# volume-em/empanada-napari

Measured on AMD Instinct MI355X. Metric: EM tiles/sec (1024^2 fp16), higher is better.
Workload: dtype f16

## Files before the change

### empanada-napari_amd/_abi.py

```python
import ctypes as C
import os

from . import build as _build

_lib = None

c_int, c_i32, c_i64, c_f32, c_f64 = C.c_int, C.c_int32, C.c_int64, C.c_float, C.c_double
vp, cp, sz = C.c_void_p, C.c_char_p, C.c_size_t


class PdlConfig(C.Structure):
    _fields_ = [
        ('num_classes', c_i32), ('stage4_stride', c_i32), ('decoder_channels', c_i32),
        ('aspp_channels', c_i32), ('n_stages', c_i32), ('low_level_stages', c_i32 * 3),
        ('low_level_proj_sem', c_i32 * 3), ('low_level_proj_ins', c_i32 * 3),
        ('atrous_rates', c_i32 * 3), ('ins_decoder', c_i32), ('num_fc', c_i32),
        ('subdivision_num_points', c_i32), ('arch', c_i32), ('fpn_dim', c_i32), ('fpn_layers', c_i32),
        ('encoder', c_i32), ('rn_stem', c_i32), ('rn_widths', c_i32 * 4), ('rn_depths', c_i32 * 4),
        ('rn_groups', c_i32 * 4), ('rn_strides', c_i32 * 4), ('rn_se', c_i32),
    ]


PROTOTYPES = {
    'emp_last_error': (cp, []),
# ... 13 lines not shown
    'emp_pdl_forward_padded': (c_int, [vp, vp, c_int, c_f32, c_f32, c_int, c_int, c_int, c_int, c_int, c_int, c_int, vp,
                                       vp, vp, vp]),
    'emp_pdl_flops': (c_f64, [vp, c_int, c_int, c_int, c_int]),
    'emp_pdl_profile': (c_int, [vp, c_int]),
    'emp_pdl_profile_read': (c_int, [vp, C.POINTER(c_f64), C.POINTER(c_f64), C.POINTER(c_int)]),
    'emp_pdl_tap': (c_int, [vp, cp, C.POINTER(vp), C.POINTER(c_i64)]),
    'emp_pdl_num_taps': (c_int, [vp]),
    'emp_pdl_tap_raw': (c_int, [vp, cp, C.POINTER(vp), C.POINTER(c_i64)]),
    'emp_pdl_tap_name': (cp, [vp, c_int]),
    'emp_copy_d2d': (c_int, [vp, vp, sz, vp]),
    'emp_conv2d_nhwc_f16': (c_int, [vp, c_int, c_int, c_int, c_int, c_int, vp, vp, vp, vp, c_int, vp, c_int, c_int,
                                    c_int, c_int, c_int, c_int, c_int, c_int, c_int, vp]),
    'emp_conv256_pack_weights': (c_int, [vp, vp, c_int, c_int, c_int, c_int, vp]),
    'emp_conv2d_grouped_nhwc_f32': (c_int, [vp, c_int, c_int, c_int, c_int, c_int, c_int, c_int, vp, vp, vp, c_int, c_int, c_int,
                                            c_int, c_int, c_int, c_int, c_int, vp]),
    'emp_conv2d_nhwc_f32': (c_int, [vp, c_int, c_int, c_int, c_int, c_int, vp, vp, vp, vp, c_int, vp, c_int, c_int,
                                    c_int, c_int, c_int, c_int, c_int, c_int, vp]),
    'emp_conv2d_nhwc_f16x3': (c_int, [vp, c_int, c_int, c_int, c_int, c_int, vp, vp, vp, vp, c_int, vp, c_int, c_int,
                                      c_int, c_int, c_int, c_int, c_int, c_int, c_int, c_int, vp]),
    'emp_conv2d_nhwc_f16x3_ex': (c_int, [vp, c_int, c_int, c_int, c_int, c_int, vp, vp, vp, vp, c_int, vp, c_int, c_int, c_int,
                                         c_int, c_int, c_int, c_int, c_int, c_int, c_int, vp, c_int, c_int, c_int, c_int, c_int,
                                         vp, vp, c_int, vp, vp]),
    'emp_sepconv_x3_pack': (c_int, [vp, vp, c_int, c_int, c_int, vp, vp, vp]),
    'emp_sepconv_x3_nhwc_f32': (c_int, [vp, c_int, c_int, c_int, c_int, c_int, vp, vp, vp, c_int, c_int, vp, c_int, vp, vp, c_int, vp,
                                        c_int, vp]),
    'emp_hl32_from_f32': (c_int, [vp, vp, c_i64, c_int, c_int, c_int, vp]),
    'emp_hl32_to_f32': (c_int, [vp, vp, c_i64, c_int, c_int, c_int, vp]),
    'emp_x3p_pack_weights': (c_int, [vp, vp, c_int, c_int, vp]),
    'emp_conv2d_hl32_f16x3': (c_int, [vp, c_int, c_int, c_int, c_int, c_int, vp, vp, vp, vp, c_int, c_int, vp, c_int, c_int, c_int,
                                      c_int, c_int, c_int, c_int, c_int, c_int, vp]),
    'emp_conv2d_hl32_f16x3_ksplit': (c_int, [vp, c_int, c_int, c_int, c_int, c_int, vp, vp, vp, vp, c_int, c_int, vp, c_int, c_int, vp, c_int, c_int,
                                             c_int, c_int, c_int, c_int, c_int, c_int, c_int, vp, c_i64, vp]),
    'emp_conv1x1_dual_nhwc_f16': (c_int, [vp, c_int, c_int, c_int, c_int, c_int, vp, c_int, c_int, c_int, c_int, c_int, vp, vp, vp,
                                  c_int, c_int, c_int, c_int, vp]),
    'emp_dwconv_nhwc_f16': (c_int, [vp, c_int, c_int, c_int, c_int, c_int, vp, c_int, vp, c_int, vp]),
    'emp_sepconv5x5_pack_pw': (c_int, [vp, c_int, c_int, c_int, vp, vp]),
    'emp_sepconv5x5_nhwc_f16': (c_int, [vp, c_int, c_int, c_int, c_int, c_int, vp, vp, vp, c_int, c_int, vp,
                                        c_int, vp, vp, c_int, vp, vp]),
    'emp_sepconvp_pack_dw': (c_int, [vp, c_int, c_int, vp, vp]),
    'emp_sepconvp_pack_pw': (c_int, [vp, c_int, c_int, c_int, vp, vp]),
    'emp_sepconvp_nhwc_f16': (c_int, [vp, c_int, c_int, c_int, c_int, c_int, c_int, vp, vp, vp, c_int, c_int, vp,
                                      c_int, vp, vp, c_int, vp, vp]),
    'emp_sepconvp_ws_pack_pw': (c_int, [vp, c_int, c_int, c_int, vp, vp]),
    'emp_sepconvp_ws_nhwc_f16': (c_int, [vp, c_int, c_int, c_int, c_int, c_int, c_int, vp, vp, vp, c_int, c_int, vp,
                                         c_int, vp, vp, c_int, vp, vp]),
    'emp_sepconv3x3_nhwc_f16': (c_int, [vp, c_int, c_int, c_int, c_int, c_int, vp, vp, vp, c_int, c_int, vp, c_int, vp]),
    'emp_sm_create': (vp, [c_i64, c_i64, c_f64, c_f64, c_int]),
    'emp_sm_destroy': (None, [vp]),
    'emp_sm_push_slice_runs': (c_int, [vp, vp, c_i64, c_i64, c_i64]),
    'emp_sm_push_slices_runs': (c_int, [vp, c_i64, vp, vp, c_i64, c_i64]),
    'emp_sm_push_slice_objects': (c_int, [vp, c_i64, vp, vp, vp, vp, vp]),
    'emp_sm_num_slices': (c_i64, [vp]),
    'emp_lsa_maximize': (c_int, [vp, c_i64, c_i64, vp, vp]),
    'emp_lsa_maximize_sparse': (c_int, [c_i64, c_i64, c_i64, vp, vp, vp, vp, vp]),
    'emp_sm_prepare': (c_int, [vp, c_i64, c_i64]),
    'emp_sm_state_size': (c_int, [vp, c_i64, vp, vp]),
    'emp_sm_export_state': (c_int, [vp, c_i64, vp, vp, vp, vp]),
    'emp_sm_import_state': (c_int, [vp, c_i64, c_i64, vp, vp, vp, c_i64, c_int]),
    'emp_sm_begin_backward': (c_int, [vp]),
    'emp_sm_step_begin': (c_int, [vp, c_i64, C.POINTER(c_int), C.POINTER(c_int)]),
    'emp_sm_iou': (vp, [vp]),
    'emp_sm_step_apply': (c_int, [vp, vp, vp, c_i64]),
    'emp_sm_run': (c_int, [vp, c_i64, c_int, c_i64, c_int, vp]),
    'emp_sm_solver_stats': (c_int, [vp, C.POINTER(c_i64), C.POINTER(c_i64)]),
    'emp_sm_pending_shape': (c_int, [vp, vp, vp]),
    'emp_sm_tracker_init': (c_int, [vp, c_int, c_i64, c_i64, c_i64]),
    'emp_sm_track': (c_int, [vp, c_i64, c_i64]),
    'emp_sm_track_range': (c_int, [vp, c_i64, c_i64, c_i64]),
    'emp_sm_tracker_finish': (c_int, [vp]),
    'emp_sm_num_tracks': (c_i64, [vp]),
    'emp_sm_track_info': (c_int, [vp, c_i64, C.POINTER(c_i64), C.POINTER(c_i64), C.POINTER(c_i64)]),
    'emp_sm_track_runs': (c_int, [vp, c_i64, vp, vp]),
    'emp_sm_tracks_info': (c_int, [vp, vp, vp, vp, C.POINTER(c_i64)]),
    'emp_sm_tracks_runs': (c_int, [vp, vp, vp]),
    'emp_sm_slice_num_objects': (c_i64, [vp, c_i64]),
    'emp_sm_slice_object_info': (c_int, [vp, c_i64, c_i64, C.POINTER(c_i64), C.POINTER(c_i64), C.POINTER(c_i64)]),
    'emp_sm_slice_object_runs': (c_int, [vp, c_i64, c_i64, vp, vp]),
    'emp_logits_to_prob': (c_int, [vp, vp, c_int, c_int, c_int, c_int, vp]),
    'emp_median_slices': (c_int, [C.POINTER(vp), c_int, vp, sz, vp]),
    'emp_median_recursive': (c_int, [vp, vp, c_int, c_int, c_int, vp, sz, vp]),
    'emp_instance_cells_work_bytes': (sz, [c_int, c_int, c_int]),
    'emp_instance_cells': (c_int, [vp, vp, c_int, c_int, c_int, c_f32, c_int, c_int, c_int, vp, vp, vp, c_int, vp, vp]),
    'emp_panoptic_merge_work_bytes': (sz, [c_int, c_int, c_int]),
    'emp_ccl8_work_bytes': (sz, [c_int, c_int, c_int]),
    'emp_ccl8': (c_int, [vp, c_int, c_int, c_int, vp, vp, vp, vp]),
    'emp_force_connected_work_bytes': (sz, [c_int, c_int, c_int]),
    'emp_force_connected': (c_int, [vp, c_int, c_int, c_int, C.POINTER(c_i32), c_int, c_i64, vp, vp, vp]),
    'emp_ccl26': (c_int, [vp, c_int, c_int, c_int, vp, vp, vp, vp]),
    'emp_morph_cross3d': (c_int, [vp, vp, c_int, c_int, c_int, c_int, vp]),
    'emp_fill_holes_slices': (c_int, [vp, c_i64, c_i64, c_i64]),
    'emp_rle_extract_work_bytes': (sz, [c_int, c_int, c_int]),
    'emp_rle_extract': (c_int, [vp, c_int, c_int, c_int, vp, vp, c_int, vp, vp]),
    'emp_ccl_range': (c_int, [vp, c_int, c_int, c_int, c_int, c_int, c_i64, c_i64, vp, vp, vp, vp]),
    'emp_rle_extract_range': (c_int, [vp, c_int, c_int, c_int, c_int, c_i64, c_i64, vp, vp, c_int, vp, vp]),
    'emp_rle_fill': (c_int, [vp, vp, vp, c_i64, vp, c_i64, c_int, vp]),
    'emp_rle_fill_ordered': (c_int, [vp, vp, vp, vp, c_i64, vp, c_i64, c_int, vp, vp]),
    'emp_rle_pair_intersections': (c_int, [vp, vp, vp, vp, c_i64, vp]),
    'emp_ranges_vote': (c_int, [vp, c_i64, c_int, vp, C.POINTER(c_i64)]),
    'emp_gather_segments_i64': (c_int, [vp, vp, vp, vp, vp, vp, c_i64, vp, vp]),
    'emp_panoptic_merge': (c_int, [vp, vp, c_int, c_int, c_int, c_int, c_f32, C.POINTER(c_i32), c_int, c_i64, c_i64,
                                   c_i64, c_int, vp, vp, vp]),
    'emp_label_overlap_work_bytes': (sz, [c_i64]),
    'emp_label_overlap_reset': (c_int, [vp, c_i64, vp]),
    'emp_label_overlap_accumulate': (c_int, [vp, c_int, vp, c_int, c_i64, vp, c_i64, vp, C.POINTER(c_int)]),
    'emp_label_overlap_grow': (c_int, [vp, c_i64, vp, c_i64, vp, C.POINTER(c_int)]),
    'emp_label_overlap_finalize': (c_int, [vp, c_i64, vp, vp, c_i64, C.POINTER(c_i64), vp]),
    'emp_overlap_match': (c_int, [c_i64, vp, vp, vp, c_int, vp, vp, C.POINTER(c_i64), vp, vp, C.POINTER(c_i64), vp, vp, vp, vp,
                                  C.POINTER(c_i64)]),
    'emp_label_table_work_bytes': (sz, [c_i64]),
    'emp_label_table_reset': (c_int, [vp, c_i64, vp]),
    'emp_label_table_accumulate': (c_int, [vp, c_int, c_i64, c_int, c_int, c_int, c_int, vp, c_i64, vp, C.POINTER(c_int)]),
    'emp_label_table_grow': (c_int, [vp, c_i64, vp, c_i64, vp, C.POINTER(c_int)]),
    'emp_label_table_finalize': (c_int, [vp, c_i64, vp, vp, vp, c_i64, C.POINTER(c_i64), vp]),
    'emp_label_map_build': (c_int, [vp, vp, c_i64, vp, vp, c_i64, vp]),
    'emp_label_apply_map': (c_int, [vp, c_int, vp, c_int, vp, c_i64, c_int, c_int, c_int, c_int, vp, vp, c_i64, vp]),
    'emp_morph_tile_shape': (c_int, [c_int, c_int, c_int, C.POINTER(c_int), C.POINTER(c_int), C.POINTER(c_int)]),
    'emp_morph_labels': (c_int, [vp, c_int, c_int, c_int, c_int, c_int, c_int, c_int, vp, vp, c_i64, vp, vp, c_int, vp, c_i64, vp,
                                 C.POINTER(c_int)]),
    'emp_fill_holes_tile_shape': (c_int, [c_int, C.POINTER(c_int), C.POINTER(c_int), C.POINTER(c_int)]),
    'emp_fill_holes_labels': (c_int, [vp, c_int, c_int, c_int, c_int, c_int, c_int, c_i64, vp, vp, vp, c_i64, vp, vp, c_int, vp, vp, c_i64,
                                      vp, C.POINTER(c_int)]),
}


class EmpError(RuntimeError):
    pass


def lib_path():
    return _build.LIB


def load(build_if_missing=False):
    global _lib
    if _lib is not None:
        return _lib
    import torch
    path = lib_path()
    if not os.path.exists(path):
        if build_if_missing:
            _build.build_all()
        else:
            raise EmpError(f'{path} not found: run `python __graft_entry__.py` (build()) first; '
                           'the HIP engine has no CPU fallback')
    lib = C.CDLL(path)
    for name, (res, args) in PROTOTYPES.items():
        try:
            fn = getattr(lib, name)
        except AttributeError as e:
            raise EmpError(f'{path} does not export {name}') from e
        fn.restype = res
        fn.argtypes = args
    _lib = lib
    return lib


def check(rc, what=''):
    if rc != 0:
        msg = load().emp_last_error()
        raise EmpError(f'{what} failed ({rc}): {msg.decode() if msg else "?"}')


def ptr(t):
    return None if t is None else C.c_void_p(t.data_ptr())


# ... 4 lines not shown
```

### empanada-napari_amd/csrc/abi.hip

```cpp
#include <stdarg.h>

#include <map>
#include <mutex>
#include <utility>
#include <vector>

#include "common.h"

namespace emp {

static thread_local char g_err[1024] = "no error";

void set_error(const char* fmt, ...) {
  va_list ap;
  va_start(ap, fmt);
  vsnprintf(g_err, sizeof(g_err), fmt, ap);
  va_end(ap);
}

const void* zero_page() {
  static void* page = nullptr;
  static std::once_flag once;
  std::call_once(once, [] {
    if (hipMalloc(&page, 2048) != hipSuccess) { page = nullptr; return; }
    if (hipMemset(page, 0, 2048) != hipSuccess) { (void)hipFree(page); page = nullptr; }
  });
  return page;
}

int ensure_dyn_lds(const void* kernel, int bytes) {
  static std::mutex mu;
  static std::map<std::pair<int, const void*>, int> done;
  int dev = 0;
  EMP_CHECK_HIP(hipGetDevice(&dev));
  std::lock_guard<std::mutex> lk(mu);
  auto it = done.find({dev, kernel});
  if (it != done.end() && it->second >= bytes) return EMP_OK;
  EMP_CHECK_HIP(hipFuncSetAttribute(kernel, hipFuncAttributeMaxDynamicSharedMemorySize, bytes));
  done[{dev, kernel}] = bytes;
  return EMP_OK;
}

}

using namespace emp;

extern "C" {

const char* emp_last_error(void) { return g_err; }
int emp_abi_version(void) { return 5; }

int emp_device_count(void) {
  int n = 0;
  hipError_t e = hipGetDeviceCount(&n);
  if (e != hipSuccess) {
    set_error("hipGetDeviceCount: %s", hipGetErrorString(e));
    return EMP_ERR_HIP;
  }
  return n;
}

int emp_copy_d2d(void* d_dst, const void* d_src, size_t bytes, void* stream) {
  EMP_REQUIRE(d_dst && d_src, "copy_d2d: null pointer");
  EMP_CHECK_HIP(hipMemcpyAsync(d_dst, d_src, bytes, hipMemcpyDeviceToDevice, (hipStream_t)stream));
  return EMP_OK;
}

int emp_conv2d_nhwc_f16(const void* d_in, int N, int H, int W, int Cin, int in_ld, const void* d_w,
                        const float* d_bias, const float* d_bias_n, const void* d_res, int res_ld, void* d_out,
                        int out_ld, int Cout, int KH, int KW, int stride, int pad, int dil, int relu, int variant,
                        void* stream) {
  EMP_REQUIRE(d_in && d_w && d_out, "conv2d: null pointer");
  EMP_REQUIRE(N > 0 && H > 0 && W > 0 && KH > 0 && KW > 0 && stride > 0 && dil > 0 && pad >= 0, "conv2d: bad geometry");
  EMP_REQUIRE(variant >= 0 && (variant & 15) <= 3 && ((variant >> 4) & 15) <= 7 && ((variant >> 8) & 255) <= 64 && (variant >> 16) <= 31, "conv2d: bad variant %d", variant);
  ConvParams p{};
  p.in = (const half_t*)d_in;
  p.wgt = (const half_t*)d_w;
  p.bias = d_bias;
  p.bias_n = d_bias_n;
  p.res = (const half_t*)d_res;
  p.res_ld = res_ld;
  p.out = (half_t*)d_out;
  p.zero = (const half_t*)zero_page();
  EMP_REQUIRE(p.zero != nullptr, "conv2d: could not allocate the zero page");
  p.N = N; p.H = H; p.W = W; p.Cin = Cin; p.in_ld = in_ld;
  p.Cout = Cout; p.KH = KH; p.KW = KW; p.stride = stride; p.pad = pad; p.dil = dil;
  p.Ho = (H + 2 * pad - dil * (KH - 1) - 1) / stride + 1;
  p.Wo = (W + 2 * pad - dil * (KW - 1) - 1) / stride + 1;
  EMP_REQUIRE(p.Ho > 0 && p.Wo > 0, "conv2d: empty output");
  p.out_ld = out_ld;
  p.act = relu;
  p.ps_cout = 0;
  p.M = N * p.Ho * p.Wo;
  return launch_conv_igemm(p, variant, (hipStream_t)stream);
}

int emp_conv256_pack_weights(const void* d_w, void* d_packed, int Cout, int KT, int Cin, int Cin2, void* stream) {
  return conv256_pack_weights((const half_t*)d_w, (half_t*)d_packed, Cout, KT, Cin, Cin2, (hipStream_t)stream);
}

int emp_conv2d_nhwc_f32(const float* d_in, int N, int H, int W, int Cin, int in_ld, const float* d_w, const float* d_bias,
                        const float* d_bias_n, const float* d_res, int res_ld, float* d_out, int out_ld, int Cout, int KH,
                        int KW, int stride, int pad, int dil, int act, void* stream) {
  EMP_REQUIRE(d_in && d_w && d_out, "conv2d_f32: null pointer");
  EMP_REQUIRE(N > 0 && H > 0 && W > 0 && KH > 0 && KW > 0 && stride > 0 && dil > 0 && pad >= 0, "conv2d_f32: bad geometry");
  Conv32 p{};
  p.in = d_in; p.in_ld = in_ld; p.w = d_w; p.bias = d_bias; p.bias_n = d_bias_n; p.res = d_res; p.res_ld = res_ld;
  p.out = d_out; p.out_ld = out_ld;
  p.N = N; p.H = H; p.W = W; p.Cin = Cin; p.Cout = Cout; p.KH = KH; p.KW = KW; p.stride = stride; p.pad = pad; p.dil = dil;
  p.Ho = (H + 2 * pad - dil * (KH - 1) - 1) / stride + 1;
  p.Wo = (W + 2 * pad - dil * (KW - 1) - 1) / stride + 1;
  EMP_REQUIRE(p.Ho > 0 && p.Wo > 0 && out_ld >= Cout && (d_res == nullptr || res_ld >= Cout), "conv2d_f32: bad output geometry");
  p.act = act;
  return launch_conv32(p, (hipStream_t)stream);
}

int emp_conv2d_nhwc_f16x3(const float* d_in, int N, int H, int W, int Cin, int in_ld, const float* d_w, const float* d_bias,
                          const float* d_bias_n, const float* d_res, int res_ld, float* d_out, int out_ld, int Cout, int KH,
                          int KW, int stride, int pad, int dil, int act, int groups, int cin_g, void* stream) {
  EMP_REQUIRE(d_in && d_w && d_out, "conv2d_f16x3: null pointer");
  EMP_REQUIRE(N > 0 && H > 0 && W > 0 && KH > 0 && KW > 0 && stride > 0 && dil > 0 && pad >= 0 && groups >= 1, "conv2d_f16x3: bad geometry");
  Conv32 p{};
  p.in = d_in; p.in_ld = in_ld; p.w = d_w; p.bias = d_bias; p.bias_n = d_bias_n; p.res = d_res; p.res_ld = res_ld;
  p.out = d_out; p.out_ld = out_ld;
  p.N = N; p.H = H; p.W = W; p.Cin = Cin; p.Cout = Cout; p.KH = KH; p.KW = KW; p.stride = stride; p.pad = pad; p.dil = dil;
  p.Ho = (H + 2 * pad - dil * (KH - 1) - 1) / stride + 1;
  p.Wo = (W + 2 * pad - dil * (KW - 1) - 1) / stride + 1;
  EMP_REQUIRE(p.Ho > 0 && p.Wo > 0 && out_ld >= groups * Cout && (d_res == nullptr || res_ld >= Cout), "conv2d_f16x3: bad output geometry");
  p.act = act;
  p.x3 = 1;
  if (groups > 1) { p.groups = groups; p.cin_g = cin_g; }
  return launch_conv32(p, (hipStream_t)stream);
}

int emp_conv2d_nhwc_f16x3_ex(const float* d_in, int N, int H, int W, int Cin, int in_ld, const float* d_w, const float* d_bias,
                             const float* d_bias_n, const float* d_res, int res_ld, void* d_out, int out_ld, int out_fmt, int Cout, int KH,
                             int KW, int stride, int pad, int dil, int act, int wmode, const float* d_in2, int H2, int W2, int Cin2,
                             int in2_ld, int stride2, const float* d_head_w, const float* d_head_b, int head_c, float* d_head_out,
                             void* stream) {
  EMP_REQUIRE(d_in && d_w && (d_out || d_head_w), "conv2d_f16x3_ex: null pointer");
  EMP_REQUIRE(N > 0 && H > 0 && W > 0 && KH > 0 && KW > 0 && stride > 0 && dil > 0 && pad >= 0 && wmode >= 0 && (wmode & 3) <= 2 && wmode < 8,
              "conv2d_f16x3_ex: bad geometry (wmode 0 fp32 weights, 1 split pairs, 2 pairs + LDS-DMA image; + 4: split-K allowed)");
  const bool ksplit = (wmode & 4) != 0;
  wmode &= 3;
  hipStream_t s = (hipStream_t)stream;
  Conv32 p{};
  p.in = d_in; p.in_ld = in_ld; p.w = d_w; p.bias = d_bias; p.bias_n = d_bias_n; p.res = d_res; p.res_ld = res_ld;
  p.out = (float*)d_out; p.out_ld = out_ld; p.out_fmt = out_fmt;
// ... 238 lines not shown
```

### empanada-napari_amd/csrc/common.h

```cpp
#pragma once
#include <hip/hip_runtime.h>
#include <stdint.h>
#include <stdio.h>
#include <string>

#include "../../include/empanada_hip.h"

typedef _Float16 half_t;
typedef _Float16 f16x8 __attribute__((ext_vector_type(8)));
typedef _Float16 f16x4 __attribute__((ext_vector_type(4)));
typedef _Float16 f16x2 __attribute__((ext_vector_type(2)));
typedef float f32x4 __attribute__((ext_vector_type(4)));

namespace emp {

void set_error(const char* fmt, ...);

#define EMP_CHECK_HIP(expr)                                                        \
  do {                                                                             \
    hipError_t _e = (expr);                                                        \
    if (_e != hipSuccess) {                                                        \
      emp::set_error("%s:%d: %s -> %s", __FILE__, __LINE__, #expr, hipGetErrorString(_e)); \
      return EMP_ERR_HIP;                                                          \
    }                                                                              \
// ... 88 lines not shown
int launch_sepconv5(const half_t* in, int N, int H, int W, int C, int in_ld, const half_t* dww, const half_t* pww_packed,
                    const float* bias, int Cout, int act, half_t* out, int out_ld, const float* head_w,
                    const float* head_b, int head_c, float* hout, int64_t plane, const half_t* zero, hipStream_t s,
                    int ks = 5);
bool sepconvp_supported(int C, int Cout, int head_c);
bool sepconvp_wsplit_supported(int Cout);
int launch_sepconvp_pack_pw(const float* w, int pw_ld, int C, int Cout, half_t* packed, hipStream_t s, int wsplit = 0);
int launch_sepconvp_pack_dw(const float* w, int ks, int C, float* packed, hipStream_t s);
int launch_sepconvp(const half_t* in, int N, int H, int W, int C, int in_ld, const float* dww_packed, const half_t* pww_packed,
                    const float* bias, int Cout, int act, half_t* out, int out_ld, const float* head_w,
                    const float* head_b, int head_c, float* hout, int64_t plane, const half_t* zero, hipStream_t s,
                    int ks = 5, int wsplit = 0);
int launch_head1x1(const half_t* in, int N, int P, int K, int in_ld, const float* w, const float* b, int C,
                   float* out, int64_t plane_size, const int32_t* scatter_idx, hipStream_t s);
int launch_bilinear_ac_f32_nchw(const float* in, int NC, int h, int w, float* out, int scale, hipStream_t s);
int launch_zero(void* p, size_t bytes, hipStream_t s);

struct Conv32 {
  const float* in; int in_ld;
  const float* w; const float* bias; const float* bias_n;
  const float* res; int res_ld;
  float* out; int out_ld;
  int N, H, W, Cin, Cout, KH, KW, stride, pad, dil, Ho, Wo;
  int act;
  int ps_cout;
  int groups;
  int cin_g;
  int x3;
  const float* in2; int in2_ld, Cin2, H2, W2, stride2;
  const float* head_w; float* head_part; int head_c;
  int x3_mt, x3_nt, x3_mtx;
  const float* zero;
  const uint32_t* wpair;
  const half_t* wimg;
  int in_fmt, out_fmt, res_fmt;
  const half_t* wimgp;
  float* out2; int out2_ld, split2;
  int x3p_kg;
  float* kpart; int64_t kpart_bytes; int ksplit, x3_ksteps;
};
constexpr int64_t X3_KPART_BYTES = 64ll << 20;
int launch_conv32(const Conv32& p, hipStream_t s);
int launch_conv16x3(const Conv32& p, hipStream_t s);
int launch_split_pairs(const float* w, uint32_t* out, int64_t n, hipStream_t s);
int64_t x3_weight_image_halfs(int Cout, int K, int Cin);
int launch_x3_weight_image(const float* w, half_t* out, int Cout, int K, hipStream_t s);
bool conv16x3p_supported(const Conv32& p);
int launch_conv16x3p(const Conv32& p, hipStream_t s);
int64_t x3p_image_halfs(int Cout, int K);
int x3p_kgroup(int KT, int Cin);
int launch_x3p_pack(const float* w, half_t* out, int Cout, int K, hipStream_t s, int KT = 0, int Cin = 0, int kg = 0);
int launch_hl32_from_f32(const float* in, half_t* out, int64_t rows, int C, int in_ld, int out_ld, hipStream_t s);
int launch_hl32_to_f32(const half_t* in, float* out, int64_t rows, int C, int in_ld, int out_ld, hipStream_t s);
int launch_avgpool_hl32(const half_t* in, int N, int HW, int C, int in_ld, float* out, hipStream_t s);
bool sepconv_x3_supported(int C, int Cout, int head_c, int ks);
int64_t sepx3_pw_halfs(int C, int Cout);
int launch_sepx3_pack_pw(const float* w, int pw_ld, int C, int Cout, half_t* packed, hipStream_t s);
int launch_sepx3_pack_dw(const float* w , int ks, int C, int ld, float* packed, hipStream_t s);
int launch_sepconv_x3(const float* in, int N, int H, int W, int C, int in_ld, const float* dww, const half_t* pww, const float* bias,
                      int Cout, int act, float* out, int out_ld, const float* head_w, const float* head_b, int head_c, float* hout,
                      int64_t plane, hipStream_t s, int ks = 5);
int conv16x3_cout_tiles(int Cout);
int launch_head_finish_f32(const float* part, int tiles, int N, int P, int C, const float* b, float* out, hipStream_t s);
int launch_stem3x3s2_f32(const void* img, int dtype, float sub, float mul, int N, int H, int W, int vh, int vw,
                         const float* w , const float* b, int C, float* out, int out_ld, hipStream_t s);
int launch_gate_mul_f32(float* x, int x_ld, const float* g, int g_ld, int64_t rows, int C, hipStream_t s);
int launch_stem7x7_f32(const void* img, int dtype, float sub, float mul, int N, int H, int W, int vh, int vw,
                       const float* w , const float* b , float* out, hipStream_t s);
int launch_maxpool3x3s2_f32(const float* in, int N, int H, int W, int C, float* out, hipStream_t s);
int launch_dwconv_f32(const float* in, int N, int H, int W, int C, int in_ld, const float* w , int K, float* out,
                      int out_ld, hipStream_t s);
int launch_bilinear_ac_f32_nhwc(const float* in, int N, int h, int w, int C, int in_ld, float* out, int H, int W, int out_ld,
                                hipStream_t s);
int launch_avgpool_f32(const float* in, int N, int HW, int C, int in_ld, float* out, hipStream_t s);
int launch_fuse_combine_f32(const float* a, const float* b, const float* c, float ca, float cb, float cc, int mode, int N,
                            int H, int W, int C, float* out, hipStream_t s);
int launch_head1x1_f32(const float* in, int N, int P, int K, int in_ld, const float* w, const float* b, int C, float* out,
                       int64_t plane_size, const int32_t* scatter_idx, hipStream_t s);
int launch_point_features_f32(const float* feat, int N, int fh, int fw, int C, int feat_ld, const float* coarse, int ncls,
                              const int32_t* idx, int P, int H2, int W2, float* x0, float* x1, int ld, hipStream_t s);

size_t topk_work_bytes(int N, int64_t plane);
int launch_upsample2x_keys(const float* in, int N, int C, int h, int w, float* out, uint32_t* keys, hipStream_t s);
int launch_topk_smallest(const uint32_t* keys, int N, int64_t plane, int k, void* work, size_t work_bytes,
                         int32_t* idx_out, hipStream_t s);
int launch_point_features(const half_t* feat, int N, int fh, int fw, int C, int feat_ld, const float* coarse,
                          int ncls, const int32_t* idx, int P, int H2, int W2, half_t* x0, half_t* x1, int ld,
                          hipStream_t s);

bool pr_mlp_supported(int C, int ld, int ncls, int num_fc);
int launch_pr_mlp(const half_t* feat, int N, int fh, int fw, int C, int feat_ld, const float* coarse, int ncls,
                  const int32_t* idx, int P, int H2, int W2, const half_t* const* fc_w, const float* const* fc_b,
                  int num_fc, int ld, const float* pred_w, const float* pred_b, float* out, int64_t plane, hipStream_t s);


}
```

### empanada-napari_amd/csrc/pdl_net.hip

```cpp
#include <string.h>

#include <array>
#include <map>
#include <memory>
#include <string>
#include <vector>

#include "common.h"

namespace emp {

namespace {

struct HostParam {
  std::vector<int64_t> shape;
  std::vector<float> w, b;
  bool set = false;
};

struct Act {
  half_t* p = nullptr;
  int N = 0, H = 0, W = 0, C = 0, ld = 0;
  size_t off = 0;
};
// ... 5 lines not shown
  int cout = 0, cin = 0, cin_pad = 0, kh = 1, kw = 1;
  int cin2 = 0, cin2_pad = 0;
  bool wsplit = false;
};

inline int round_up(int a, int b) { return (a + b - 1) / b * b; }

}
}

using namespace emp;

struct emp_pdl {
  emp_pdl_config cfg;
  int aspp_ch = 256, dec_ch = 256, ncls = 1;
  std::vector<std::string> param_names;
  std::map<std::string, HostParam> params;
  bool finalized = false;
  FILE* layer_log = [] { const char* e = getenv("EMP_LAYER_LOG"); return e ? fopen(e, "w") : (FILE*)nullptr; }();
  bool fuse_stem = [] { const char* e = getenv("EMP_FUSE_STEM"); return !(e && e[0] == '0'); }();
  bool fuse_ds = [] { const char* e = getenv("EMP_FUSE_DS"); return !(e && e[0] == '0'); }();
  bool fuse_b2b = [] { const char* e = getenv("EMP_FUSE_B2B"); return !(e && e[0] == '0'); }();
  bool pack256 = [] { const char* e = getenv("EMP_CONV256_PACK"); return !(e && e[0] == '0'); }();
  bool fuse_proj = [] { const char* e = getenv("EMP_FUSE_PROJ"); return !(e && e[0] == '0'); }();
  bool fuse_aspp = [] { const char* e = getenv("EMP_FUSE_ASPP"); return !(e && e[0] == '0'); }();
  bool fuse_sepconv = [] { const char* e = getenv("EMP_FUSE_SEPCONV"); return !(e && e[0] == '0'); }();
  bool fuse_pr = [] { const char* e = getenv("EMP_FUSE_PR"); return !(e && e[0] == '0'); }();
  int precise_sepconv = [] { const char* e = getenv("EMP_PRECISE_SEPCONV"); return e ? atoi(e) : 1; }();
  bool precise_wsplit = [] { const char* e = getenv("EMP_PRECISE_WSPLIT"); return !(e && e[0] == '0'); }();
  bool precise_fsplit = [] { const char* e = getenv("EMP_PRECISE_FSPLIT"); return !(e && e[0] == '0'); }();
  int sepconv_min_tiles = [] { const char* e = getenv("EMP_SEPCONV_MIN_TILES"); return e ? atoi(e) : 256; }();

  int precision = [] {
    const char* e = getenv("EMP_PRECISION");
    if (e && (!strcmp(e, "fp16") || !strcmp(e, "16"))) return 0;
    if (e && (!strcmp(e, "fp32") || !strcmp(e, "32"))) return 1;
    return 2;
  }();
  bool fp32_graph() const { return precision != 0; }
  bool x3_fuse_ds = [] { const char* e = getenv("EMP_X3_FUSE_DS"); return !(e && e[0] == '0'); }();
  bool x3_fuse_head = [] { const char* e = getenv("EMP_X3_FUSE_HEAD"); return !(e && e[0] == '0'); }();
  bool x3_planes = [] { const char* e = getenv("EMP_X3_PLANES"); return !(e && e[0] == '0'); }();
  int x3_planes_min_tiles = [] { const char* e = getenv("EMP_X3_PLANES_MIN_TILES"); return e ? atoi(e) : 128; }();
  bool x3_planes_ready = false;
  bool x3_ksplit = [] { const char* e = getenv("EMP_X3_KSPLIT"); return !(e && e[0] == '0'); }();
  float* x3_kpart = nullptr;
  bool x3_small_aspp = [] { const char* e = getenv("EMP_X3_SMALL_ASPP"); return !(e && e[0] == '0'); }();
  bool x3_fuse_stem = [] { const char* e = getenv("EMP_X3_FUSE_STEM"); return !(e && e[0] == '0'); }();
  bool x3_merge_proj = [] { const char* e = getenv("EMP_X3_MERGE_PROJ"); return !(e && e[0] == '0'); }();
  bool x3_merge_aspp = [] { const char* e = getenv("EMP_X3_MERGE_ASPP"); return !(e && e[0] == '0'); }();
  bool x3_fuse_sep = [] { const char* e = getenv("EMP_X3_FUSE_SEP"); return !(e && e[0] == '0'); }();
  int x3_sep_min_tiles = [] { const char* e = getenv("EMP_X3_SEP_MIN_TILES"); return e ? atoi(e) : 1; }();
  struct SepX3 { float* dw = nullptr; half_t* pw = nullptr; int C = 0, Cout = 0, ks = 0; };
  std::map<std::string, SepX3> sepx3;
  bool regnet_grouped = [] { const char* e = getenv("EMP_REGNET_GROUPED"); return !(e && e[0] == '0'); }();
  int64_t regnet_group_tiles = [] { const char* e = getenv("EMP_REGNET_GROUP_TILES"); return e ? atoll(e) : 2048ll; }();
  struct W32 { float* w = nullptr; float* b = nullptr; int cout = 0, cin = 0, cin16 = 0, kh = 1, kw = 1; uint32_t* wp = nullptr; int cin2 = 0, cin2_16 = 0; half_t* wimg = nullptr; half_t* wimgp = nullptr; int x3p_kg = 0; };
  std::map<std::string, W32> w32;
  std::map<std::string, std::pair<float*, size_t>> pool32;
  std::map<std::string, std::array<int, 4>> geom32;

  std::map<std::string, DevConv> convs;
  std::map<std::string, float*> f32w;
  std::map<std::string, half_t*> f16w;
  std::map<std::string, std::vector<float>> fusew;
  std::vector<void*> owned;

  char* arena = nullptr;
  size_t arena_cap = 0, arena_used = 0;
  int pN = 0, pH = 0, pW = 0, pRS = 0;
  int capN = 0;
  std::map<std::string, Act> acts;
  std::vector<std::string> act_order;
  std::map<std::string, std::pair<size_t, size_t>> raw;
  double flops = 0.0;
  size_t image_bytes = 0;
  bool profile = false;
  std::vector<std::pair<hipEvent_t, hipEvent_t>> prof_events;
  size_t prof_used = 0;
  double prof_flops = 0.0;
  int64_t par_limit = [] { const char* e = getenv("EMP_PAR_DECODERS"); return e ? atoll(e) : (int64_t)4 << 20; }();
  hipStream_t aux = nullptr;
  hipEvent_t ev_fork = nullptr, ev_join = nullptr;

  ~emp_pdl() {
    for (void* p : owned) (void)hipFree(p);
    for (auto& kv : pool32) (void)hipFree(kv.second.first);
    if (arena) (void)hipFree(arena);
    if (layer_log) fclose(layer_log);
    for (auto& e : prof_events) { (void)hipEventDestroy(e.first); (void)hipEventDestroy(e.second); }
    if (ev_fork) (void)hipEventDestroy(ev_fork);
    if (ev_join) (void)hipEventDestroy(ev_join);
    if (aux) (void)hipStreamDestroy(aux);
  }
};

namespace {

const int kLayers[4] = {3, 4, 6, 3};
const int kPlanes[4] = {64, 128, 256, 512};

bool precise_layer(const emp_pdl* n, const std::string& pre) {
  const int mode = n->precise_sepconv;
  if (mode <= 0) return false;
  if (mode == 2) return true;
  const char* dec = n->cfg.ins_decoder ? "instance_decoder." : "semantic_decoder.";
  const bool head = pre.compare(0, 11, "ins_center.") == 0, fuse = pre.compare(0, strlen(dec), dec) == 0;
  if (mode == 3) return head;
  if (mode == 4) return fuse;
  if ((mode == 6 || (mode == 1 && n->cfg.arch == 1)) && pre.compare(0, 7, "ins_xy.") == 0) return true;
  return head || fuse;
}

bool precise_node(const emp_pdl* n, const std::string& name) {
  const int mode = n->precise_sepconv;
  if (mode == 2 || mode == 5) return true;
  if (mode != 1 && mode != 6) return false;
  const char* fp = n->cfg.ins_decoder ? "instance_fpn." : "semantic_fpn.";
  return name.compare(0, strlen(fp), fp) == 0;
}

bool wsplit_on(const emp_pdl* n) {
  const int mode = n->precise_sepconv;
  return n->cfg.arch == 1 && n->precise_wsplit && (mode == 1 || mode == 2 || mode == 5 || mode == 6);
}

bool fsplit_on(const emp_pdl* n, const std::string& name) {
  const int F = n->cfg.fpn_dim;
  return wsplit_on(n) && n->precise_fsplit && n->fuse_sepconv && precise_node(n, name) && sepconvp_supported(2 * F, F, 0);
}

void expect(emp_pdl* n, const std::string& name) {
  n->param_names.push_back(name);
  n->params[name] = HostParam();
}

bool regnet_has_shortcut(const emp_pdl_config& c, int si, int b) {
  if (b > 1) return false;
  const int w_in = si == 1 ? c.rn_stem : c.rn_widths[si - 2];
  return w_in != c.rn_widths[si - 1] || c.rn_strides[si - 1] > 1;
}

void build_param_list(emp_pdl* n) {
  const emp_pdl_config& c = n->cfg;
  if (c.encoder == 1) {
    expect(n, "encoder.stem.cbr.0");
    for (int si = 1; si <= 4; ++si)
      for (int b = 1; b <= c.rn_depths[si - 1]; ++b) {
        const std::string p = "encoder.stage" + std::to_string(si) + ".block" + std::to_string(b);
        expect(n, p + ".bottleneck.a.0");
        expect(n, p + ".bottleneck.b.0");
        if (c.rn_se) {
          expect(n, p + ".bottleneck.se.se.0");
          expect(n, p + ".bottleneck.se.se.2");
        }
        expect(n, p + ".bottleneck.c.0");
        if (regnet_has_shortcut(c, si, b)) expect(n, p + ".downsample.conv.0");
      }
  } else {
    expect(n, "encoder.conv1");
    for (int li = 1; li <= 4; ++li)
      for (int b = 0; b < kLayers[li - 1]; ++b) {
        std::string p = "encoder.layer" + std::to_string(li) + "." + std::to_string(b);
        expect(n, p + ".conv1");
        expect(n, p + ".conv2");
        expect(n, p + ".conv3");
// ... 332 lines not shown
  if (c.arch == 0) {
    const int h5 = ph[4], w5 = pw[4];
    add_raw(n, pl, "pooled", (size_t)N * 2048 * 4);
    add_raw(n, pl, "pool_part", (size_t)avgpool_scratch_floats(N, 2048) * 4);
    const char* decs[2] = {"semantic_decoder", "instance_decoder"};
    for (int d = 0; d < (c.ins_decoder ? 2 : 1); ++d) {
      std::string p = decs[d];
      add_raw(n, pl, p + ".poolfeat", (size_t)N * n->aspp_ch * 4);
      add_raw(n, pl, p + ".bias_n", (size_t)N * n->aspp_ch * 4);
      add_act(n, pl, p + ".aspp.cat", N, h5, w5, 4 * n->aspp_ch);
      add_act(n, pl, p + ".aspp", N, h5, w5, n->aspp_ch);
      int xch = n->aspp_ch;
      for (int i = 0; i < c.n_stages; ++i) {
        const int st = c.low_level_stages[i];
        const int lp = d == 0 ? c.low_level_proj_sem[i] : c.low_level_proj_ins[i];
        const int cpad = round_up(xch + lp, 64);
        std::string q = p + ".stage" + std::to_string(i);
        add_act(n, pl, q + ".cat", N, ph[st], pw[st], cpad);
        add_act(n, pl, q + ".dw", N, ph[st], pw[st], cpad);
        add_act(n, pl, q + ".out", N, ph[st], pw[st], n->dec_ch);
        xch = n->dec_ch;
      }
    }
    const int st_last = c.low_level_stages[c.n_stages - 1];
    hq = ph[st_last]; wq = pw[st_last];
    EMP_REQUIRE(hq * 4 == H && wq * 4 == W, "the last decoder stage must be at 1/4 resolution (got %dx%d)", hq, wq);

  } else {
    EMP_REQUIRE(H % 128 == 0 && W % 128 == 0, "BiFPN forward: H=%d W=%d must be multiples of 128", H, W);
    const int F = c.fpn_dim;
    hq = ph[1]; wq = pw[1];
    add_act(n, pl, "p2f", N, ph[1], pw[1], F);
    int lh[5], lw[5];
    for (int i = 0; i < 3; ++i) { lh[i] = ph[2 + i]; lw[i] = pw[2 + i]; }
    lh[3] = lh[2] / 2; lw[3] = lw[2] / 2; lh[4] = lh[3] / 2; lw[4] = lw[3] / 2;
    const char* dn[2] = {"semantic", "instance"};
    for (int d = 0; d < (c.ins_decoder ? 2 : 1); ++d) {
      std::string fp = std::string(dn[d]) + "_fpn";
      add_act(n, pl, fp + ".p6pre", N, lh[2], lw[2], F);
      add_act(n, pl, fp + ".in.P6", N, lh[3], lw[3], F);
      add_act(n, pl, fp + ".in.P7", N, lh[4], lw[4], F);
      for (int li = 0; li < c.fpn_layers; ++li) {
        std::string L = fp + ".l" + std::to_string(li);
        for (int lv = 0; lv < 5; ++lv) {
          std::string q = L + ".P" + std::to_string(3 + lv);
          if (li == 0 && lv < 3) { add_act(n, pl, q + ".rtd", N, lh[lv], lw[lv], F); add_act(n, pl, q + ".rbu", N, lh[lv], lw[lv], F); }
          const int FZ = fsplit_on(n, fp + ".") ? 2 * F : F;
          add_act(n, pl, q + ".fuse", N, lh[lv], lw[lv], FZ);
          if (lv > 0) add_act(n, pl, q + ".fuseb", N, lh[lv], lw[lv], FZ);
          add_act(n, pl, q + ".dw", N, lh[lv], lw[lv], F);
          add_act(n, pl, q + ".td", N, lh[lv], lw[lv], F);
          add_act(n, pl, q + ".bu", N, lh[lv], lw[lv], F);
        }
      }
      std::string dp = std::string(dn[d]) + "_decoder";
      int hh = lh[4], ww = lw[4];
      for (int i = 0; i < 5; ++i) {
        hh *= 2; ww *= 2;
        add_act(n, pl, dp + ".cat" + std::to_string(i), N, hh, ww, 2 * F);
      }
      add_act(n, pl, dp + ".dw", N, hq, wq, 2 * F);
      add_act(n, pl, dp + ".out", N, hq, wq, F);
    }
  }
  const char* heads[3] = {"semantic_head", "ins_center", "ins_xy"};
  const int hc[3] = {n->ncls, 1, 2};
  for (int k = 0; k < 3; ++k) {
    std::string p = heads[k];
    add_act(n, pl, p + ".dw", N, hq, wq, n->dec_ch);
    add_act(n, pl, p + ".pw", N, hq, wq, n->dec_ch);
    add_raw(n, pl, p + ".out", (size_t)N * hc[k] * hq * wq * 4);
  }
  const int P = c.subdivision_num_points;
  const int ldp = round_up(n->dec_ch + n->ncls, 64);
  int64_t plane_max = 0;
  {
    int hh = hq, ww = wq;
    for (int s = 0; s < RS; ++s) {
      hh *= 2; ww *= 2;
      if (s + 1 < RS) add_raw(n, pl, "pr.sem" + std::to_string(s), (size_t)N * n->ncls * hh * ww * 4);
      plane_max = (int64_t)hh * ww;
    }
  }
  add_raw(n, pl, "pr.keys", (size_t)N * plane_max * 4);
  add_raw(n, pl, "pr.topk", topk_work_bytes(N, plane_max));
  add_raw(n, pl, "pr.idx", (size_t)N * P * 4);
  add_raw(n, pl, "pr.x0", (size_t)N * P * ldp * 2);
  add_raw(n, pl, "pr.x1", (size_t)N * P * ldp * 2);

  const size_t need = pl.off;
  if (need > n->arena_cap) {
    if (n->arena) EMP_CHECK_HIP(hipFree(n->arena));
    n->arena = nullptr;
    n->arena_cap = 0;
    hipError_t e = hipMalloc((void**)&n->arena, need);
    if (e != hipSuccess) {
      set_error("arena: hipMalloc(%zu bytes) failed: %s", need, hipGetErrorString(e));
      return EMP_ERR_NOMEM;
    }
    n->arena_cap = need;
  }
  EMP_CHECK_HIP(hipMemsetAsync(n->arena, 0, need, stream));
  n->arena_used = need;
  for (auto& kv : n->acts) kv.second.p = (half_t*)(n->arena + kv.second.off);
  n->pN = N; n->pH = H; n->pW = W; n->pRS = RS;
  n->capN = N;
  return EMP_OK;
}

void rebatch(emp_pdl* n, int N) {
  for (auto& kv : n->acts) kv.second.N = N;
  n->pN = N;
}

template <typename T>
T* rawp(emp_pdl* n, const std::string& name) {
  return (T*)(n->arena + n->raw.at(name).first);
}

int conv(emp_pdl* n, const std::string& wname, const Act& in, int in_coff, const Act& out, int out_coff, int stride,
         int pad, int dil, int act, const Act* res, const float* bias_n, hipStream_t s, int ps_cout = 0,
         const Act* in2 = nullptr, int stride2 = 1, const Act* out2 = nullptr, int out2_coff = 0, int split = 0,
         const std::string* next_name = nullptr, const Act* next_out = nullptr, bool* fused_next = nullptr,
         const Act* out3 = nullptr, int out3_coff = 0, int split3 = 0) {
  DevConv& dc = n->convs.at(wname);
  ConvParams p{};
  if (out3) {
    EMP_REQUIRE(out2 && out3->N == out.N && out3->H == out.H && out3->W == out.W && out3_coff + dc.cout - split3 <= out3->ld,
                "%s: third destination mismatch", wname.c_str());
    p.out3 = out3->p + out3_coff; p.out3_ld = out3->ld; p.split3 = split3;
  }
  if (out2) {
    EMP_REQUIRE(out2->N == out.N && out2->H == out.H && out2->W == out.W &&
                    out2_coff + (out3 ? split3 : dc.cout) - split <= out2->ld,
                "%s: second destination mismatch", wname.c_str());
    p.out2 = out2->p + out2_coff; p.out2_ld = out2->ld; p.split = split;
  }
  if (in2) {
    EMP_REQUIRE(dc.cin2_pad > 0 && dc.cin2_pad <= in2->ld && in2->N == in.N, "%s: second source mismatch", wname.c_str());
    p.in2 = in2->p; p.Cin2 = dc.cin2_pad; p.in2_ld = in2->ld; p.H2 = in2->H; p.W2 = in2->W; p.stride2 = stride2;
  } else {
    EMP_REQUIRE(dc.cin2_pad == 0, "%s: packed for two sources", wname.c_str());
  }
  p.in = in.p + in_coff;
  p.wgt = dc.w;
  p.bias = dc.b;
  p.bias_n = bias_n;
  p.res = res ? res->p : nullptr;
  p.res_ld = res ? res->ld : 0;
  p.out = out.p + out_coff;
  p.zero = rawp<half_t>(n, "zero");
  p.N = in.N; p.H = in.H; p.W = in.W; p.Cin = dc.cin_pad; p.in_ld = in.ld;
  p.Cout = dc.cout; p.KH = dc.kh; p.KW = dc.kw; p.stride = stride; p.pad = pad; p.dil = dil;
  p.Ho = (in.H + 2 * pad - dil * (dc.kh - 1) - 1) / stride + 1;
  p.Wo = (in.W + 2 * pad - dil * (dc.kw - 1) - 1) / stride + 1;
  const int up = ps_cout ? 2 : 1;
  EMP_REQUIRE(p.Ho * up == out.H && p.Wo * up == out.W && in.N == out.N, "%s: output shape mismatch (%dx%d vs %dx%d)",
              wname.c_str(), p.Ho * up, p.Wo * up, out.H, out.W);
  EMP_REQUIRE(in_coff + dc.cin_pad <= in.ld && out_coff + (ps_cout ? ps_cout : (out2 ? split : dc.cout)) <= out.ld,
              "%s: channel slice out of range", wname.c_str());
  p.out_ld = out.ld;
  p.act = act;
  p.ps_cout = ps_cout;
  p.M = p.N * p.Ho * p.Wo;
  double next_flops = 0.0;
  if (fused_next) *fused_next = false;
  if (next_name && n->fuse_b2b) {
// ... 384 lines not shown
      n->flops += 2.0 * 25.0 * (double)N * cb.H * cb.W * (xch + n->convs.at(p + ".project." + std::to_string(i) + ".0").cout);
      {
        const DevConv& pwc = n->convs.at(fz + "1");
        const Act& so = A(q + ".out");
        if (n->fuse_sepconv && precise_layer(n, p + ".fuse." + std::to_string(i) + ".0") && n->f16w.count(fz + "1.packedp") &&
            pwc.cin_pad == cb.ld && so.ld == pwc.cout && sepconvp_supported(cb.ld, pwc.cout, 0)) {
          RC(launch_sepconvp(cb.p, N, cb.H, cb.W, cb.ld, cb.ld, n->f32w.at(fz + "0.f32"), n->f16w.at(fz + "1.packedp"), pwc.b,
                             pwc.cout, 1, so.p, so.ld, nullptr, nullptr, 0, nullptr, 0, rawp<half_t>(n, "zero"), s));
          n->flops += 2.0 * (double)N * cb.H * cb.W * pwc.cout * (double)pwc.cin;
          if (n->layer_log) fprintf(n->layer_log, "sepconvp,%s,%d,%d,%d,5,1,1,0,%d\n", fz.c_str(), N * cb.H * cb.W, cb.ld, pwc.cout, N * cb.H * cb.W);
        } else if (n->fuse_sepconv && n->f16w.count(fz + "1.packed") && pwc.cin_pad == cb.ld && so.ld == pwc.cout &&
            sepconv5_supported(cb.ld, pwc.cout, 0)) {
          RC(launch_sepconv5(cb.p, N, cb.H, cb.W, cb.ld, cb.ld, n->f16w.at(fz + "0"), n->f16w.at(fz + "1.packed"), pwc.b,
                             pwc.cout, 1, so.p, so.ld, nullptr, nullptr, 0, nullptr, 0, rawp<half_t>(n, "zero"), s));
          n->flops += 2.0 * (double)N * cb.H * cb.W * pwc.cout * (double)pwc.cin;
          if (n->layer_log) fprintf(n->layer_log, "sepconv,%s,%d,%d,%d,5,1,1,0,%d\n", fz.c_str(), N * cb.H * cb.W, cb.ld, pwc.cout, N * cb.H * cb.W);
        } else {
          RC(launch_dwconv(cb.p, N, cb.H, cb.W, cb.ld, cb.ld, n->f16w.at(fz + "0"), 5, A(q + ".dw").p, cb.ld,
                           rawp<half_t>(n, "zero"), s));
          RC(conv(n, fz + "1", A(q + ".dw"), 0, so, 0, 1, 0, 1, true, nullptr, nullptr, s));
        }
      }
      x = q + ".out";
      xch = n->dec_ch;
    }
    dec_out[d] = x;
  }
  }
  if (!c.ins_decoder) dec_out[1] = dec_out[0];
  const Act& semx = A(dec_out[0]);
  const Act& insx = A(dec_out[1]);
  const int hq = semx.H, wq = semx.W;

  const char* heads[3] = {"semantic_head", "ins_center", "ins_xy"};
  const int hc[3] = {n->ncls, 1, 2};
  float* head_out[3];
  for (int k = 0; k < 3; ++k) {
    hipStream_t s = (par && k > 0) ? n->aux : s_main;
    std::string p = heads[k];
    const Act& xin = k == 0 ? semx : insx;
    n->flops += 2.0 * 25.0 * (double)N * hq * wq * n->dec_ch;
    float* dst = rawp<float>(n, p + ".out");
    if (k == 1 && !interp) dst = o_ctr;
    if (k == 2 && !interp) dst = o_off;
    head_out[k] = dst;
    const DevConv& pwc = n->convs.at(p + ".head.0.0.sepconv.1");
    if (n->fuse_sepconv && precise_layer(n, p + ".head.0.0") && n->f16w.count(p + ".head.0.0.sepconv.1.packedp") &&
        xin.C == n->dec_ch && pwc.cin_pad == n->dec_ch && pwc.cout == n->dec_ch && hc[k] <= 2 &&
        sepconvp_supported(n->dec_ch, pwc.cout, hc[k])) {
      RC(launch_sepconvp(xin.p, N, hq, wq, n->dec_ch, xin.ld, n->f32w.at(p + ".head.0.0.sepconv.0.f32"),
                         n->f16w.at(p + ".head.0.0.sepconv.1.packedp"), pwc.b, pwc.cout, 1, nullptr, 0, n->f32w.at(p + ".head.1.w"),
                         n->f32w.at(p + ".head.1.b"), hc[k], dst, (int64_t)hq * wq, rawp<half_t>(n, "zero"), s, 5, pwc.wsplit ? 1 : 0));
      n->flops += 2.0 * (double)N * hq * wq * pwc.cout * (double)pwc.cin;
      if (n->layer_log) fprintf(n->layer_log, "sepheadp,%s,%d,%d,%d,5,1,1,0,%d\n", p.c_str(), N * hq * wq, n->dec_ch, pwc.cout, N * hq * wq);
    } else if (n->fuse_sepconv && n->f16w.count(p + ".head.0.0.sepconv.1.packed") && xin.C == n->dec_ch &&
        pwc.cin_pad == n->dec_ch && pwc.cout == n->dec_ch && hc[k] <= 2 &&
        sepconv5_supported(n->dec_ch, pwc.cout, hc[k])) {
      RC(launch_sepconv5(xin.p, N, hq, wq, n->dec_ch, xin.ld, n->f16w.at(p + ".head.0.0.sepconv.0"),
                         n->f16w.at(p + ".head.0.0.sepconv.1.packed"), pwc.b, pwc.cout, 1, nullptr, 0, n->f32w.at(p + ".head.1.w"), n->f32w.at(p + ".head.1.b"), hc[k],
                         dst, (int64_t)hq * wq, rawp<half_t>(n, "zero"), s));
      n->flops += 2.0 * (double)N * hq * wq * pwc.cout * (double)pwc.cin;
      if (n->layer_log) fprintf(n->layer_log, "sephead,%s,%d,%d,%d,5,1,1,0,%d\n", p.c_str(), N * hq * wq, n->dec_ch, pwc.cout, N * hq * wq);
    } else {
      RC(launch_dwconv(xin.p, N, hq, wq, n->dec_ch, xin.ld, n->f16w.at(p + ".head.0.0.sepconv.0"), 5, A(p + ".dw").p,
                       n->dec_ch, rawp<half_t>(n, "zero"), s));
      RC(conv(n, p + ".head.0.0.sepconv.1", A(p + ".dw"), 0, A(p + ".pw"), 0, 1, 0, 1, true, nullptr, nullptr, s));
      RC(launch_head1x1(A(p + ".pw").p, N, hq * wq, n->dec_ch, n->dec_ch, n->f32w.at(p + ".head.1.w"),
                        n->f32w.at(p + ".head.1.b"), hc[k], dst, (int64_t)hq * wq, nullptr, s));
    }
    n->flops += 2.0 * (double)N * hq * wq * n->dec_ch * hc[k];
  }
  if (interp) {
    hipStream_t s = par ? n->aux : s_main;
    RC(launch_bilinear_ac_f32_nchw(head_out[1], N * 1, hq, wq, o_ctr, 4, s));
    RC(launch_bilinear_ac_f32_nchw(head_out[2], N * 2, hq, wq, o_off, 4, s));
  }
  if (par) EMP_CHECK_HIP(hipEventRecord(n->ev_join, n->aux));

  const int P = c.subdivision_num_points;
  const int ldp = round_up(n->dec_ch + n->ncls, 64);
  const float* coarse = head_out[0];
  const float* cur = coarse;
  int hh = hq, ww = wq;
  uint32_t* keys = rawp<uint32_t>(n, "pr.keys");
  int32_t* idx = rawp<int32_t>(n, "pr.idx");
  half_t* X[2] = {rawp<half_t>(n, "pr.x0"), rawp<half_t>(n, "pr.x1")};
  for (int st = 0; st < RS; ++st) {
    float* nxt = (st + 1 < RS) ? rawp<float>(n, "pr.sem" + std::to_string(st)) : o_sem;
    RC(launch_upsample2x_keys(cur, N, n->ncls, hh, ww, nxt, keys, s));
    hh *= 2; ww *= 2;
    const int64_t plane = (int64_t)hh * ww;
    const int k = (int)(plane < P ? plane : P);
    RC(launch_topk_smallest(keys, N, plane, k, rawp<char>(n, "pr.topk"), n->raw.at("pr.topk").second, idx, s));
    if (n->fuse_pr && pr_mlp_supported(n->dec_ch, ldp, n->ncls, c.num_fc)) {
      const half_t* fw_[4];
      const float* fb_[4];
      for (int f = 0; f < c.num_fc; ++f) {
        const DevConv& dc = n->convs.at("semantic_pr.point_head.fc_layers." + std::to_string(f) + ".0");
        fw_[f] = dc.w; fb_[f] = dc.b;
        n->flops += 2.0 * (double)N * k * dc.cout * (double)dc.cin;
      }
      RC(launch_pr_mlp(semx.p, N, hq, wq, n->dec_ch, semx.ld, coarse, n->ncls, idx, k, hh, ww, fw_, fb_, c.num_fc, ldp,
                       n->f32w.at("pr.predictor.w"), n->f32w.at("pr.predictor.b"), nxt, plane, s));
      n->flops += 2.0 * (double)N * k * ldp * n->ncls;
      cur = nxt;
      continue;
    }
    RC(launch_point_features(semx.p, N, hq, wq, n->dec_ch, semx.ld, coarse, n->ncls, idx, k, hh, ww, X[0], X[1], ldp, s));
    Act xa[2];
    for (int j = 0; j < 2; ++j) {
      xa[j].p = X[j]; xa[j].N = 1; xa[j].H = 1; xa[j].W = N * k; xa[j].C = ldp; xa[j].ld = ldp;
    }
    int curx = 0;
    for (int f = 0; f < c.num_fc; ++f) {
      RC(conv(n, "semantic_pr.point_head.fc_layers." + std::to_string(f) + ".0", xa[curx], 0, xa[curx ^ 1], 0, 1, 0, 1,
              true, nullptr, nullptr, s));
      curx ^= 1;
    }
    RC(launch_head1x1(X[curx], N, k, ldp, ldp, n->f32w.at("pr.predictor.w"), n->f32w.at("pr.predictor.b"), n->ncls, nxt,
                      plane, idx, s));
    n->flops += 2.0 * (double)N * k * ldp * n->ncls;
    cur = nxt;
  }
  if (par) EMP_CHECK_HIP(hipStreamWaitEvent(s_main, n->ev_join, 0));
  return EMP_OK;
}

struct T32 { float* p = nullptr; int N = 0, H = 0, W = 0, C = 0, ld = 0; int fmt = 0; };

int buf32(emp_pdl* n, const std::string& key, size_t floats, float** out) {
  auto it = n->pool32.find(key);
  if (it == n->pool32.end() || it->second.second < floats) {
    if (it != n->pool32.end()) { EMP_CHECK_HIP(hipFree(it->second.first)); n->pool32.erase(it); }
    float* d = nullptr;
    hipError_t e = hipMalloc((void**)&d, floats * sizeof(float) + 64);
    if (e != hipSuccess) {
      set_error("fp32 mode: hipMalloc(%zu bytes) for '%s' failed: %s", floats * sizeof(float), key.c_str(), hipGetErrorString(e));
      return EMP_ERR_NOMEM;
    }
    EMP_CHECK_HIP(hipMemset(d, 0, floats * sizeof(float)));
    n->pool32[key] = {d, floats};
    *out = d;
    return EMP_OK;
  }
  *out = it->second.first;
  return EMP_OK;
}

int t32(emp_pdl* n, const std::string& key, int N, int H, int W, int C, T32* t) {
  t->N = N; t->H = H; t->W = W; t->C = C; t->ld = C;
  return buf32(n, key, (size_t)N * H * W * C, &t->p);
}

int pack32(emp_pdl* n, const std::string& name, int cin_to = 0, const HostParam* src = nullptr) {
  const HostParam& hp = src ? *src : n->params.at(name);
  EMP_REQUIRE(hp.shape.size() == 4 || hp.shape.size() == 3, "%s: conv weight must be 3-d or 4-d", name.c_str());
  emp_pdl::W32 w;
  w.cout = (int)hp.shape[0];
  w.cin = (int)hp.shape[1];
  w.kh = hp.shape.size() == 4 ? (int)hp.shape[2] : 1;
  w.kw = hp.shape.size() == 4 ? (int)hp.shape[3] : 1;
  w.cin16 = cin_to ? cin_to : round_up(w.cin, 16);
  EMP_REQUIRE(w.cin16 >= w.cin && w.cin16 % 16 == 0, "%s: bad channel padding", name.c_str());
  const int kt = w.kh * w.kw;
  std::vector<float> pk((size_t)w.cout * kt * w.cin16, 0.f);
  for (int o = 0; o < w.cout; ++o)
    for (int i = 0; i < w.cin; ++i)
      for (int t = 0; t < kt; ++t) pk[((size_t)o * kt + t) * w.cin16 + i] = hp.w[((size_t)o * w.cin + i) * kt + t];
  void* d;
  int rc = dev_upload(n, pk.data(), pk.size() * sizeof(float), &d);
  if (rc) return rc;
  w.w = (float*)d;
  rc = dev_upload(n, hp.b.data(), hp.b.size() * sizeof(float), &d);
  if (rc) return rc;
  w.b = (float*)d;
  n->w32[name] = w;
// ... 644 lines not shown
        for (int i = 1; i <= 3; ++i) {
          const int r = c.atrous_rates[i - 1];
          RC32(c32(n, p + ".aspp.convs." + std::to_string(i) + ".0", p5, 0, A(p + ".aspp.cat"), i * n->aspp_ch, 1, r, r, 1, nullptr, nullptr, s));
        }
      }
      RC32(mk(p + ".aspp", p5.H, p5.W, n->aspp_ch));
      RC32(c32(n, p + ".aspp.project.0", A(p + ".aspp.cat"), 0, A(p + ".aspp"), 0, 1, 0, 1, 1, nullptr, bias_n, s));
      std::string xx = p + ".aspp";
      int xch = n->aspp_ch;
      for (int i = 0; i < c.n_stages; ++i) {
        const T32 low = A(pyr[c.low_level_stages[i]]);
        const int lp = d == 0 ? c.low_level_proj_sem[i] : c.low_level_proj_ins[i];
        const int cpad = round_up(xch + lp, n->precision == 2 ? 32 : 16);
        const std::string q = p + ".stage" + std::to_string(i);
        RC32(mk(q + ".cat", low.H, low.W, cpad));
        const T32 xa = A(xx);
        RC32(launch_bilinear_ac_f32_nhwc(xa.p, N, xa.H, xa.W, xch, xa.ld, A(q + ".cat").p, low.H, low.W, cpad, s));
        if (!proj_done[i]) RC32(c32(n, p + ".project." + std::to_string(i) + ".0", low, 0, A(q + ".cat"), xch, 1, 0, 1, 1, nullptr, nullptr, s));
        RC32(mk(q + ".out", low.H, low.W, n->dec_ch));
        bool fused = false;
        RC32(sep_x3(p + ".fuse." + std::to_string(i) + ".0.sepconv", A(q + ".cat"), 1, A(q + ".out").p, A(q + ".out").ld, nullptr, nullptr, 0, nullptr, &fused));
        if (!fused) {
          RC32(mk(q + ".dw", low.H, low.W, cpad));
          RC32(dw(A(q + ".cat"), p + ".fuse." + std::to_string(i) + ".0.sepconv.0", 5, A(q + ".dw")));
          RC32(c32(n, p + ".fuse." + std::to_string(i) + ".0.sepconv.1", A(q + ".dw"), 0, A(q + ".out"), 0, 1, 0, 1, 1, nullptr, nullptr, s));
        }
        xx = q + ".out";
        xch = n->dec_ch;
      }
      dec_out[d] = xx;
    }
  }
  if (!c.ins_decoder) dec_out[1] = dec_out[0];
  const T32 semx = A(dec_out[0]), insx = A(dec_out[1]);
  const int hq = semx.H, wq = semx.W;
  EMP_REQUIRE(hq * 4 == H && wq * 4 == W, "the decoder output must be at 1/4 resolution (got %dx%d)", hq, wq);
  const char* heads[3] = {"semantic_head", "ins_center", "ins_xy"};
  const int hc[3] = {n->ncls, 1, 2};
  float* head_out[3];
  for (int k = 0; k < 3; ++k) {
    const std::string p = heads[k];
    const T32& xin = k == 0 ? semx : insx;
    float* dst;
    RC32(buf32(n, p + ".out", (size_t)N * hc[k] * hq * wq, &dst));
    if (k == 1 && !interp) dst = o_ctr;
    if (k == 2 && !interp) dst = o_off;
    head_out[k] = dst;
    {
      bool fused = false;
      RC32(sep_x3(p + ".head.0.0.sepconv", xin, 1, nullptr, 0, n->f32w.at(p + ".head.1.w"), n->f32w.at(p + ".head.1.b"), hc[k], dst, &fused));
      if (fused) {
        n->flops += 2.0 * (double)N * hq * wq * n->dec_ch * hc[k];
        continue;
      }
    }
    RC32(mk(p + ".dw", hq, wq, n->dec_ch));
    RC32(dw(xin, p + ".head.0.0.sepconv.0", 5, A(p + ".dw")));
    if (n->precision == 2 && n->x3_fuse_head && hc[k] <= 4) {
      const int tiles = conv16x3_cout_tiles(n->dec_ch);
      float* part;
      RC32(buf32(n, p + ".part", (size_t)tiles * N * hq * wq * hc[k], &part));
      RC32(c32(n, p + ".head.0.0.sepconv.1", A(p + ".dw"), 0, A(p + ".dw"), 0, 1, 0, 1, 1, nullptr, nullptr, s, 0, 1,
               n->f32w.at(p + ".head.1.w"), part, hc[k]));
      RC32(launch_head_finish_f32(part, tiles, N, hq * wq, hc[k], n->f32w.at(p + ".head.1.b"), dst, s));
    } else {
      RC32(mk(p + ".pw", hq, wq, n->dec_ch));
      RC32(c32(n, p + ".head.0.0.sepconv.1", A(p + ".dw"), 0, A(p + ".pw"), 0, 1, 0, 1, 1, nullptr, nullptr, s));
      RC32(launch_head1x1_f32(A(p + ".pw").p, N, hq * wq, n->dec_ch, n->dec_ch, n->f32w.at(p + ".head.1.w"), n->f32w.at(p + ".head.1.b"),
                              hc[k], dst, (int64_t)hq * wq, nullptr, s));
    }
    n->flops += 2.0 * (double)N * hq * wq * n->dec_ch * hc[k];
  }
  if (interp) {
    RC32(launch_bilinear_ac_f32_nchw(head_out[1], N * 1, hq, wq, o_ctr, 4, s));
    RC32(launch_bilinear_ac_f32_nchw(head_out[2], N * 2, hq, wq, o_off, 4, s));
  }
  const int P = c.subdivision_num_points;
  const int ldp = round_up(n->dec_ch + n->ncls, 16);
  const float* coarse = head_out[0];
  const float* cur = coarse;
  int hh = hq, ww = wq;
  int64_t plane_max = (int64_t)hq * wq;
  for (int st = 0; st < RS; ++st) plane_max *= 4;
  float* fkeys;
  RC32(buf32(n, "pr.keys", (size_t)N * plane_max, &fkeys));
  float* ftopk;
  const size_t topk_bytes = topk_work_bytes(N, plane_max);
  RC32(buf32(n, "pr.topk", (topk_bytes + 3) / 4, &ftopk));
  float* fidx;
  RC32(buf32(n, "pr.idx", (size_t)N * P, &fidx));
  T32 X[2];
  for (int j = 0; j < 2; ++j) {
    X[j].N = 1; X[j].H = 1; X[j].W = N * P; X[j].C = ldp; X[j].ld = ldp;
    RC32(buf32(n, j ? "pr.x1" : "pr.x0", (size_t)N * P * ldp, &X[j].p));
  }
  for (int st = 0; st < RS; ++st) {
    float* nxt = o_sem;
    if (st + 1 < RS) RC32(buf32(n, "pr.sem" + std::to_string(st), (size_t)N * n->ncls * hh * ww * 4, &nxt));
    RC32(launch_upsample2x_keys(cur, N, n->ncls, hh, ww, nxt, (uint32_t*)fkeys, s));
    hh *= 2; ww *= 2;
    const int64_t plane = (int64_t)hh * ww;
    const int k = (int)(plane < P ? plane : P);
    RC32(launch_topk_smallest((const uint32_t*)fkeys, N, plane, k, (char*)ftopk, topk_bytes, (int32_t*)fidx, s));
    RC32(launch_point_features_f32(semx.p, N, hq, wq, n->dec_ch, semx.ld, coarse, n->ncls, (const int32_t*)fidx, k, hh, ww, X[0].p,
                                   X[1].p, ldp, s));
    T32 xa[2] = {X[0], X[1]};
    xa[0].W = xa[1].W = N * k;
    int curx = 0;
    for (int f = 0; f < c.num_fc; ++f) {
      RC32(c32(n, "semantic_pr.point_head.fc_layers." + std::to_string(f) + ".0", xa[curx], 0, xa[curx ^ 1], 0, 1, 0, 1, 1, nullptr,
               nullptr, s));
      curx ^= 1;
    }
    RC32(launch_head1x1_f32(xa[curx].p, N, k, ldp, ldp, n->f32w.at("pr.predictor.w32"), n->f32w.at("pr.predictor.b"), n->ncls, nxt,
                            plane, (const int32_t*)fidx, s));
    n->flops += 2.0 * (double)N * k * ldp * n->ncls;
    cur = nxt;
  }
  return EMP_OK;
}

}

extern "C" {

int emp_pdl_create(const emp_pdl_config* cfg, emp_pdl_t** out) {
  EMP_REQUIRE(cfg && out, "pdl_create: null argument");
  EMP_REQUIRE(cfg->num_classes >= 1 && cfg->num_classes <= 8, "num_classes=%d unsupported", cfg->num_classes);
  EMP_REQUIRE(cfg->stage4_stride == 16 || cfg->stage4_stride == 32, "stage4_stride must be 16 or 32");
  EMP_REQUIRE(cfg->arch == 0 || cfg->arch == 1, "arch must be 0 (PanopticDeepLabPR) or 1 (PanopticBiFPNPR)");
  if (cfg->arch == 1) {
    EMP_REQUIRE(cfg->fpn_dim > 0 && cfg->fpn_dim % 64 == 0 && cfg->fpn_layers >= 1 && cfg->stage4_stride == 32,
                "BiFPN: fpn_dim must be a multiple of 64, fpn_layers >= 1, stage4_stride 32");
  } else {
  EMP_REQUIRE(cfg->n_stages >= 1 && cfg->n_stages <= 3, "n_stages=%d unsupported", cfg->n_stages);
  EMP_REQUIRE(cfg->decoder_channels % 64 == 0 && cfg->decoder_channels > 0, "decoder_channels must be a multiple of 64");
  }
  EMP_REQUIRE(cfg->num_fc >= 1 && cfg->subdivision_num_points > 0, "bad PointRend configuration");
  for (int i = 0; i < (cfg->arch == 0 ? cfg->n_stages : 0); ++i) {
    EMP_REQUIRE(cfg->low_level_stages[i] >= 1 && cfg->low_level_stages[i] <= 3, "low_level_stages[%d] out of range", i);
    EMP_REQUIRE(cfg->low_level_proj_sem[i] % 8 == 0 && (!cfg->ins_decoder || cfg->low_level_proj_ins[i] % 8 == 0),
                "projected low-level channels must be multiples of 8");
  }
  EMP_REQUIRE(cfg->encoder == 0 || cfg->encoder == 1, "encoder must be 0 (ResNet50) or 1 (RegNet)");
  if (cfg->encoder == 1) {
    EMP_REQUIRE(cfg->rn_stem > 0 && cfg->rn_stem % 4 == 0, "RegNet: stem width %d must be a positive multiple of 4", cfg->rn_stem);
    for (int i = 0; i < 4; ++i) {
      const int w = cfg->rn_widths[i], g = cfg->rn_groups[i];
      EMP_REQUIRE(w > 0 && g > 0 && w % g == 0 && (w / g) % 4 == 0 && w % 8 == 0 && cfg->rn_depths[i] >= 1 &&
                      (cfg->rn_strides[i] == 1 || cfg->rn_strides[i] == 2),
                  "RegNet stage %d: width %d (multiple of 8), groups %d (group width a multiple of 4), depth %d, stride %d", i + 1, w, g,
                  cfg->rn_depths[i], cfg->rn_strides[i]);
    }
    int os_ = 2;
    for (int i = 0; i < 4; ++i) os_ *= cfg->rn_strides[i];
    EMP_REQUIRE(cfg->rn_strides[0] == 2 && (os_ == 32 || os_ == 16) && (cfg->arch == 0 || os_ == 32),
                "RegNet: stage 1 must be at stride 4 and the encoder's output stride 16 or 32 (BiFPN: 32)");
  }
  emp_pdl* n = new (std::nothrow) emp_pdl();
  if (!n) return EMP_ERR_NOMEM;
  n->cfg = *cfg;
  n->dec_ch = cfg->arch == 1 ? cfg->fpn_dim : cfg->decoder_channels;
  n->aspp_ch = cfg->aspp_channels > 0 ? cfg->aspp_channels : cfg->decoder_channels;
  n->ncls = cfg->num_classes;
  build_param_list(n);
  *out = n;
  return EMP_OK;
}

void emp_pdl_destroy(emp_pdl_t* net) { delete net; }

int emp_pdl_num_params(const emp_pdl_t* net) { return net ? (int)net->param_names.size() : 0; }
const char* emp_pdl_param_name(const emp_pdl_t* net, int i) {
  if (!net || i < 0 || i >= (int)net->param_names.size()) return nullptr;
  return net->param_names[i].c_str();
}

int emp_pdl_set_param(emp_pdl_t* net, const char* name, const float* h_w, const int64_t* shape, int ndim,
                      const float* h_b) {
  EMP_REQUIRE(net && name && h_w && shape, "set_param: null argument");
  auto it = net->params.find(name);
  EMP_REQUIRE(it != net->params.end(), "set_param: unknown parameter '%s'", name);
  EMP_REQUIRE(ndim == 1 || ndim == 3 || ndim == 4, "set_param(%s): ndim must be 1, 3 or 4", name);
  HostParam& hp = it->second;
  hp.shape.assign(shape, shape + ndim);
  size_t cnt = 1;
// ... 408 lines not shown
```

### empanada-napari_amd/csrc/pointrend.hip

```cpp
#include "common.h"

namespace emp {
namespace {

constexpr int CHUNK = 2048;

__device__ __forceinline__ uint32_t wave_incl_scan(uint32_t v, int lane) {
#pragma unroll
  for (int o = 1; o < 64; o <<= 1) {
    uint32_t t = __shfl_up(v, o);
    if (lane >= o) v += t;
  }
  return v;
}
__device__ __forceinline__ uint32_t block_excl_scan(uint32_t v, uint32_t* sh , uint32_t* total) {
  const int lane = threadIdx.x & 63, w = threadIdx.x >> 6;
  uint32_t inc = wave_incl_scan(v, lane);
  __syncthreads();
  if (lane == 63) sh[w] = inc;
  __syncthreads();
  uint32_t base = 0;
#pragma unroll
  for (int i = 0; i < 4; ++i)
    if (i < w) base += sh[i];
  *total = sh[0] + sh[1] + sh[2] + sh[3];
  return base + inc - v;
}

__global__ void __launch_bounds__(256) upsample2x_keys_kernel(const float* __restrict__ in, int N, int C, int h, int w,
                                                              float* __restrict__ out, uint32_t* __restrict__ keys,
                                                              int64_t total) {
  const int H = 2 * h, W = 2 * w;
  for (int64_t i = (int64_t)blockIdx.x * 256 + threadIdx.x; i < total; i += (int64_t)gridDim.x * 256) {
    int ox = (int)(i % W);
    int64_t p = i / W;
    int oy = (int)(p % H);
    int n = (int)(p / H);
    float fy = 0.5f * ((float)oy + 0.5f) - 0.5f;
    float fx = 0.5f * ((float)ox + 0.5f) - 0.5f;
    fy = fy < 0.f ? 0.f : fy;
    fx = fx < 0.f ? 0.f : fx;
    int y0 = (int)fy, x0 = (int)fx;
    int y1 = y0 + (y0 < h - 1 ? 1 : 0), x1 = x0 + (x0 < w - 1 ? 1 : 0);
    float ly = fy - (float)y0, lx = fx - (float)x0;
    float hy = 1.f - ly, hx = 1.f - lx;
    float top1 = -INFINITY, top2 = -INFINITY, v0 = 0.f;
    for (int c = 0; c < C; ++c) {
      const float* b = in + ((size_t)n * C + c) * h * w;
      float v = hy * (hx * b[y0 * w + x0] + lx * b[y0 * w + x1]) + ly * (hx * b[y1 * w + x0] + lx * b[y1 * w + x1]);
      out[(((size_t)n * C + c) * H + oy) * W + ox] = v;
      if (c == 0) v0 = v;
      if (v > top1) { top2 = top1; top1 = v; } else if (v > top2) { top2 = v; }
    }
    float key = (C == 1) ? fabsf(v0) : (top1 - top2);
    keys[i] = __float_as_uint(key);
  }
}

__global__ void init_state_kernel(uint32_t* state, uint32_t* hist, int N, uint32_t k) {
  int i = blockIdx.x * 256 + threadIdx.x;
  if (i < N) { state[4 * i] = 0; state[4 * i + 1] = k; state[4 * i + 2] = 0; state[4 * i + 3] = 0; }
  if (i < N * 256) hist[i] = 0;
}

__global__ void __launch_bounds__(256) radix_hist_kernel(const uint32_t* __restrict__ keys, int64_t plane,
                                                         const uint32_t* __restrict__ state,
                                                         uint32_t* __restrict__ hist, int shift, uint32_t himask) {
  __shared__ uint32_t lh[256];
  const int n = blockIdx.y;
  lh[threadIdx.x] = 0;
  __syncthreads();
  const uint32_t prefix = state[4 * n];
  const uint32_t* kp = keys + (size_t)n * plane;
  const int64_t base = (int64_t)blockIdx.x * CHUNK;
#pragma unroll
  for (int j = 0; j < CHUNK / 256; ++j) {
    int64_t i = base + j * 256 + threadIdx.x;
    if (i < plane) {
      uint32_t k = kp[i];
      if ((k & himask) == prefix) atomicAdd(&lh[(k >> shift) & 255u], 1u);
    }
  }
  __syncthreads();
  uint32_t c = lh[threadIdx.x];
  if (c) atomicAdd(&hist[n * 256 + threadIdx.x], c);
}

__global__ void __launch_bounds__(256) radix_select_kernel(uint32_t* __restrict__ hist, uint32_t* __restrict__ state,
                                                           int shift) {
  __shared__ uint32_t sh[8];
  const int n = blockIdx.x;
  uint32_t c = hist[n * 256 + threadIdx.x];
  hist[n * 256 + threadIdx.x] = 0;
  uint32_t total;
  uint32_t ex = block_excl_scan(c, sh, &total);
  const uint32_t krem = state[4 * n + 1];
  const uint32_t prefix = state[4 * n];
  __syncthreads();
  if (c > 0 && ex < krem && krem <= ex + c) {
    state[4 * n] = prefix | ((uint32_t)threadIdx.x << shift);
    state[4 * n + 1] = krem - ex;
  }
}

__device__ __forceinline__ uint32_t count_flags(const uint32_t* kp, int64_t plane, int64_t e0, uint32_t T,
                                                uint32_t* flags_less, uint32_t* flags_eq) {
  uint32_t fl = 0, fe = 0;
#pragma unroll
  for (int j = 0; j < 8; ++j) {
    int64_t i = e0 + j;
    if (i < plane) {
      uint32_t k = kp[i];
      fl |= (uint32_t)(k < T) << j;
      fe |= (uint32_t)(k == T) << j;
    }
  }
  *flags_less = fl;
  *flags_eq = fe;
  return (uint32_t)__popc(fl) | ((uint32_t)__popc(fe) << 16);
}

__global__ void __launch_bounds__(256) compact_count_kernel(const uint32_t* __restrict__ keys, int64_t plane,
                                                            const uint32_t* __restrict__ state,
                                                            uint32_t* __restrict__ blockcnt, int nb) {
  __shared__ uint32_t sh[8];
  const int n = blockIdx.y;
  const uint32_t T = state[4 * n];
  uint32_t fl, fe;
  uint32_t c = count_flags(keys + (size_t)n * plane, plane, (int64_t)blockIdx.x * CHUNK + threadIdx.x * 8, T, &fl, &fe);
  uint32_t total;
  block_excl_scan(c, sh, &total);
  if (threadIdx.x == 0) blockcnt[(size_t)n * nb + blockIdx.x] = total;
}

__global__ void __launch_bounds__(256) compact_scan_kernel(const uint32_t* __restrict__ blockcnt,
                                                           uint32_t* __restrict__ blockoff, int nb) {
  __shared__ uint32_t sh[8];
  const int n = blockIdx.x;
  uint32_t carry_l = 0, carry_e = 0;
  for (int b0 = 0; b0 < nb; b0 += 256) {
    int b = b0 + threadIdx.x;
    uint32_t c = b < nb ? blockcnt[(size_t)n * nb + b] : 0;
    uint32_t tl, te;
    uint32_t el = block_excl_scan(c & 0xffffu, sh, &tl);
    uint32_t ee = block_excl_scan(c >> 16, sh, &te);
    if (b < nb) {
      blockoff[((size_t)n * nb + b) * 2] = carry_l + el;
      blockoff[((size_t)n * nb + b) * 2 + 1] = carry_e + ee;
    }
    carry_l += tl;
    carry_e += te;
    __syncthreads();
  }
}

__global__ void __launch_bounds__(256) compact_write_kernel(const uint32_t* __restrict__ keys, int64_t plane,
                                                            const uint32_t* __restrict__ state,
                                                            const uint32_t* __restrict__ blockoff, int nb, int k,
                                                            int32_t* __restrict__ idx_out) {
  __shared__ uint32_t sh[8];
  const int n = blockIdx.y;
  const uint32_t T = state[4 * n];
  const uint32_t krem = state[4 * n + 1];
  const uint32_t nless = (uint32_t)k - krem;
  const int64_t e0 = (int64_t)blockIdx.x * CHUNK + threadIdx.x * 8;
  uint32_t fl, fe;
  uint32_t c = count_flags(keys + (size_t)n * plane, plane, e0, T, &fl, &fe);
  uint32_t tl, te;
  uint32_t pl = block_excl_scan(c & 0xffffu, sh, &tl) + blockoff[((size_t)n * nb + blockIdx.x) * 2];
  uint32_t pe = block_excl_scan(c >> 16, sh, &te) + blockoff[((size_t)n * nb + blockIdx.x) * 2 + 1];
  int32_t* o = idx_out + (size_t)n * k;
#pragma unroll
  for (int j = 0; j < 8; ++j) {
    if (fl & (1u << j)) { o[pl++] = (int32_t)(e0 + j); }
    if (fe & (1u << j)) {
      if (pe < krem) o[nless + pe] = (int32_t)(e0 + j);
      ++pe;
    }
  }
}

__global__ void iota_kernel(int32_t* idx, int N, int k) {
  int i = blockIdx.x * 256 + threadIdx.x;
  if (i < N * k) idx[i] = i % k;
}

__global__ void __launch_bounds__(256) point_features_kernel(const half_t* __restrict__ feat, int N, int fh, int fw,
                                                             int C, int feat_ld, const float* __restrict__ coarse,
                                                             int ncls, const int32_t* __restrict__ idx, int P, int H2,
                                                             int W2, half_t* __restrict__ x0, half_t* __restrict__ x1,
                                                             int ld) {
  const int hl = threadIdx.x & 31;
  const int64_t pt = ((int64_t)blockIdx.x * 256 + threadIdx.x) >> 5;
  if (pt >= (int64_t)N * P) return;
  const int n = (int)(pt / P);
  const int id = idx[pt];
  const int iy = id / W2, ix = id - iy * W2;
  const float w_step = 1.0f / (float)W2, h_step = 1.0f / (float)H2;
  const float cx = 0.5f * w_step + w_step * (float)ix;
  const float cy = 0.5f * h_step + h_step * (float)iy;
  const float gx = 2.0f * cx - 1.0f, gy = 2.0f * cy - 1.0f;
  const float sx = ((gx + 1.f) * (float)fw - 1.f) * 0.5f;
  const float sy = ((gy + 1.f) * (float)fh - 1.f) * 0.5f;
  const float fx0 = floorf(sx), fy0 = floorf(sy);
  const int xa = (int)fx0, ya = (int)fy0, xb = xa + 1, yb = ya + 1;
  const float lx = sx - fx0, ly = sy - fy0;
  const float w00 = (1.f - lx) * (1.f - ly), w01 = lx * (1.f - ly), w10 = (1.f - lx) * ly, w11 = lx * ly;
  const bool ok00 = xa >= 0 && xa < fw && ya >= 0 && ya < fh;
  const bool ok01 = xb >= 0 && xb < fw && ya >= 0 && ya < fh;
  const bool ok10 = xa >= 0 && xa < fw && yb >= 0 && yb < fh;
  const bool ok11 = xb >= 0 && xb < fw && yb >= 0 && yb < fh;
  const int CG = C >> 3;
  half_t* r0 = x0 + (size_t)pt * ld;
  half_t* r1 = x1 + (size_t)pt * ld;
  const half_t* fb = feat + (size_t)n * fh * fw * feat_ld;
  for (int cg = hl; cg < CG; cg += 32) {
    float a[8] = {0, 0, 0, 0, 0, 0, 0, 0};
    auto accum = [&](bool ok, int yy, int xx, float wt) {
      if (ok) {
        f16x8 v = *reinterpret_cast<const f16x8*>(fb + ((size_t)yy * fw + xx) * feat_ld + cg * 8);
#pragma unroll
        for (int c = 0; c < 8; ++c) a[c] = fmaf((float)v[c], wt, a[c]);
      }
    };
    accum(ok00, ya, xa, w00);
    accum(ok01, ya, xb, w01);
    accum(ok10, yb, xa, w10);
    accum(ok11, yb, xb, w11);
    f16x8 o;
#pragma unroll
    for (int c = 0; c < 8; ++c) o[c] = (half_t)a[c];
    *reinterpret_cast<f16x8*>(r0 + cg * 8) = o;
  }
  const int tail = (ld - C) >> 3;
  if (hl < tail) {
    f16x8 o = {0, 0, 0, 0, 0, 0, 0, 0};
    if (hl == 0) {
      for (int c = 0; c < ncls && c < 8; ++c) {
        const float* cb = coarse + ((size_t)n * ncls + c) * fh * fw;
        float v = 0.f;
        if (ok00) v = fmaf(cb[ya * fw + xa], w00, v);
        if (ok01) v = fmaf(cb[ya * fw + xb], w01, v);
        if (ok10) v = fmaf(cb[yb * fw + xa], w10, v);
        if (ok11) v = fmaf(cb[yb * fw + xb], w11, v);
        o[c] = (half_t)v;
      }
    }
    *reinterpret_cast<f16x8*>(r0 + C + hl * 8) = o;
    *reinterpret_cast<f16x8*>(r1 + C + hl * 8) = o;
  }
}

template <int C>
struct PrCfg {
  static constexpr int MT = C / 128;
};

struct PrParams {
  const half_t* feat; int N, fh, fw, feat_ld;
  const float* coarse; int ncls;
  const int32_t* idx; int P, H2, W2;
  const half_t* w[4]; const float* b[4]; int num_fc;
// ... 133 lines not shown
          }
        }
        if (hf + 1 == PT / 128 && f + 1 < p.num_fc) load_weights(f + 1);
        __syncthreads();
#pragma unroll
        for (int c = 0; c < MT; ++c) {
          const int co = wave * MT * 16 + c * 16 + fq * 4;
          const float4 bv = *reinterpret_cast<const float4*>(p.b[f] + co);
#pragma unroll
          for (int q = 0; q < 8; ++q) {
            const int row = hf * 128 + q * 16 + fr;
            f16x4 o;
            o[0] = (half_t)fmaxf(acc[c][q][0] + bv.x, 0.f);
            o[1] = (half_t)fmaxf(acc[c][q][1] + bv.y, 0.f);
            o[2] = (half_t)fmaxf(acc[c][q][2] + bv.z, 0.f);
            o[3] = (half_t)fmaxf(acc[c][q][3] + bv.w, 0.f);
            *reinterpret_cast<f16x4*>(X + xoff(row, co >> 3) + (co & 7) * 2) = o;
          }
        }
      }
      __syncthreads();
    }
    for (int c = 0; c < p.ncls; ++c) {
      float wv[2][8];
#pragma unroll
      for (int jj = 0; jj < 2; ++jj) {
        const int kc = hl + 32 * jj;
        if (kc < KC) {
          const float4* wp = reinterpret_cast<const float4*>(p.pw + (size_t)c * LD + kc * 8);
          const float4 w0 = wp[0], w1 = wp[1];
          wv[jj][0] = w0.x; wv[jj][1] = w0.y; wv[jj][2] = w0.z; wv[jj][3] = w0.w;
          wv[jj][4] = w1.x; wv[jj][5] = w1.y; wv[jj][6] = w1.z; wv[jj][7] = w1.w;
        } else {
#pragma unroll
          for (int e = 0; e < 8; ++e) wv[jj][e] = 0.f;
        }
      }
      const float bias = p.pb[c];
#pragma unroll 4
      for (int j = 0; j < PT / 16; ++j) {
        const int row = hw + 16 * j;
        const int64_t pt = g0 + row;
        const bool live = pt < p.npts;
        float sacc = 0.f;
#pragma unroll
        for (int jj = 0; jj < 2; ++jj) {
          const int kc = hl + 32 * jj;
          if (kc < KC) {
            const f16x8 v = *reinterpret_cast<const f16x8*>(X + xoff(row, kc));
#pragma unroll
            for (int e = 0; e < 8; ++e) sacc = fmaf((float)v[e], wv[jj][e], sacc);
          }
        }
#pragma unroll
        for (int o = 16; o > 0; o >>= 1) sacc += __shfl_xor(sacc, o);
        if (hl == 0 && live) {
          const int n = (int)(pt / p.P);
          p.out[((size_t)n * p.ncls + c) * p.plane + (int64_t)p.idx[pt]] = sacc + bias;
        }
      }
    }
    __syncthreads();
  }
}

inline int grid_for(int64_t total, int per_block = 256, int cap = 256 * 16) {
  int64_t g = (total + per_block - 1) / per_block;
  if (g > cap) g = cap;
  if (g < 1) g = 1;
  return (int)g;
}

}

int launch_upsample2x_keys(const float* in, int N, int C, int h, int w, float* out, uint32_t* keys, hipStream_t s) {
  int64_t total = (int64_t)N * 4 * h * w;
  hipLaunchKernelGGL(upsample2x_keys_kernel, dim3(grid_for(total)), dim3(256), 0, s, in, N, C, h, w, out, keys, total);
  EMP_LAUNCH_CHECK();
  return EMP_OK;
}

size_t topk_work_bytes(int N, int64_t plane) {
  int nb = (int)cdiv64(plane, CHUNK);
  return (size_t)N * (256 + 4 + (size_t)nb * 3) * sizeof(uint32_t) + 256;
}

int launch_topk_smallest(const uint32_t* keys, int N, int64_t plane, int k, void* work, size_t work_bytes,
                         int32_t* idx_out, hipStream_t s) {
  EMP_REQUIRE(k > 0 && plane > 0, "topk: k=%d plane=%lld", k, (long long)plane);
  if ((int64_t)k >= plane) {
    EMP_REQUIRE((int64_t)k == plane, "topk: k > plane");
    hipLaunchKernelGGL(iota_kernel, dim3(cdiv(N * k, 256)), dim3(256), 0, s, idx_out, N, k);
    EMP_LAUNCH_CHECK();
    return EMP_OK;
  }
  EMP_REQUIRE(work_bytes >= topk_work_bytes(N, plane), "topk: workspace too small");
  const int nb = (int)cdiv64(plane, CHUNK);
  uint32_t* hist = (uint32_t*)work;
  uint32_t* state = hist + (size_t)N * 256;
  uint32_t* blockcnt = state + (size_t)N * 4;
  uint32_t* blockoff = blockcnt + (size_t)N * nb;
  hipLaunchKernelGGL(init_state_kernel, dim3(cdiv(N * 256, 256)), dim3(256), 0, s, state, hist, N, (uint32_t)k);
  EMP_LAUNCH_CHECK();
  for (int pass = 0; pass < 4; ++pass) {
    const int shift = 24 - 8 * pass;
    const uint32_t himask = pass == 0 ? 0u : (0xffffffffu << (shift + 8));
    hipLaunchKernelGGL(radix_hist_kernel, dim3(nb, N), dim3(256), 0, s, keys, plane, state, hist, shift, himask);
    EMP_LAUNCH_CHECK();
    hipLaunchKernelGGL(radix_select_kernel, dim3(N), dim3(256), 0, s, hist, state, shift);
    EMP_LAUNCH_CHECK();
  }
  hipLaunchKernelGGL(compact_count_kernel, dim3(nb, N), dim3(256), 0, s, keys, plane, state, blockcnt, nb);
  EMP_LAUNCH_CHECK();
  hipLaunchKernelGGL(compact_scan_kernel, dim3(N), dim3(256), 0, s, blockcnt, blockoff, nb);
  EMP_LAUNCH_CHECK();
  hipLaunchKernelGGL(compact_write_kernel, dim3(nb, N), dim3(256), 0, s, keys, plane, state, blockoff, nb, k, idx_out);
  EMP_LAUNCH_CHECK();
  return EMP_OK;
}

int launch_point_features(const half_t* feat, int N, int fh, int fw, int C, int feat_ld, const float* coarse, int ncls,
                          const int32_t* idx, int P, int H2, int W2, half_t* x0, half_t* x1, int ld, hipStream_t s) {
  EMP_REQUIRE(C % 8 == 0 && ld % 8 == 0 && ld >= C + 8 && ncls <= 8, "point_features: bad channel layout");
  EMP_REQUIRE((ld - C) / 8 <= 32, "point_features: tail too wide");
  int64_t pts = (int64_t)N * P;
  hipLaunchKernelGGL(point_features_kernel, dim3((unsigned)cdiv64(pts, 8)), dim3(256), 0, s, feat, N, fh, fw, C, feat_ld,
                     coarse, ncls, idx, P, H2, W2, x0, x1, ld);
  EMP_LAUNCH_CHECK();
  return EMP_OK;
}

bool pr_mlp_supported(int C, int ld, int ncls, int num_fc) {
  return ((C == 256 && ld == 320) || (C == 128 && ld == 192)) && ncls >= 1 && ncls <= 8 && num_fc >= 1 && num_fc <= 4;
}

int launch_pr_mlp(const half_t* feat, int N, int fh, int fw, int C, int feat_ld, const float* coarse, int ncls,
                  const int32_t* idx, int P, int H2, int W2, const half_t* const* fc_w, const float* const* fc_b,
                  int num_fc, int ld, const float* pred_w, const float* pred_b, float* out, int64_t plane,
                  hipStream_t s) {
  EMP_REQUIRE(pr_mlp_supported(C, ld, ncls, num_fc), "pr_mlp: unsupported shape C=%d ld=%d", C, ld);
  PrParams p{};
  p.feat = feat; p.N = N; p.fh = fh; p.fw = fw; p.feat_ld = feat_ld;
  p.coarse = coarse; p.ncls = ncls; p.idx = idx; p.P = P; p.H2 = H2; p.W2 = W2;
  for (int i = 0; i < num_fc; ++i) { p.w[i] = fc_w[i]; p.b[i] = fc_b[i]; }
  p.num_fc = num_fc; p.pw = pred_w; p.pb = pred_b; p.out = out; p.plane = plane;
  p.npts = (int64_t)N * P;
  p.tiles = (int)cdiv64(p.npts, 256);
  const int grid = p.tiles < 256 ? p.tiles : 256;
  const size_t lds = (size_t)256 * ld * 2;
  if (C == 256) {
    if (int rc = ensure_dyn_lds(reinterpret_cast<const void*>(&pr_mlp_kernel<256, 320>), (int)lds)) return rc;
    hipLaunchKernelGGL((pr_mlp_kernel<256, 320>), dim3(grid), dim3(512), lds, s, p);
  } else {
    if (int rc = ensure_dyn_lds(reinterpret_cast<const void*>(&pr_mlp_kernel<128, 192>), (int)lds)) return rc;
    hipLaunchKernelGGL((pr_mlp_kernel<128, 192>), dim3(grid), dim3(512), lds, s, p);
  }
  EMP_LAUNCH_CHECK();
  return EMP_OK;
}

}
```

### empanada-napari_amd/csrc/postprocess.hip

```cpp
#include "common.h"

namespace emp {
namespace {

inline int grid_for(int64_t total, int per_block = 256, int cap = 256 * 16) {
  int64_t g = (total + per_block - 1) / per_block;
  if (g > cap) g = cap;
  if (g < 1) g = 1;
  return (int)g;
}

__device__ __forceinline__ uint32_t wave_incl_scan(uint32_t v, int lane) {
#pragma unroll
  for (int o = 1; o < 64; o <<= 1) {
    uint32_t t = __shfl_up(v, o);
    if (lane >= o) v += t;
  }
  return v;
}
__device__ __forceinline__ uint32_t block_excl_scan(uint32_t v, uint32_t* sh, uint32_t* total) {
  const int lane = threadIdx.x & 63, w = threadIdx.x >> 6;
  uint32_t inc = wave_incl_scan(v, lane);
  __syncthreads();
  if (lane == 63) sh[w] = inc;
// ... 250 lines not shown
          if (s2 > best_hi) continue;
          const float d = __builtin_sqrtf(s2);
          const int idx = __float_as_int(c.z);
          if (d < best || (d == best && idx < id)) { best = d; best_s = s2; best_hi = s2 * 1.000004f; id = idx; }
        }
      };
      for (int r = 0;; ++r) {
        const int y0 = by - r, y1 = by + r, x0 = bx - r, x1 = bx + r;
        if (y0 < 0 && y1 >= GH && x0 < 0 && x1 >= GW) break;
        const int xa = x0 > 0 ? x0 : 0, xb = x1 < GW - 1 ? x1 : GW - 1;
        if (y0 >= 0) scan(start[y0 * GW + xa], start[y0 * GW + xb + 1]);
        if (r > 0 && y1 < GH) scan(start[y1 * GW + xa], start[y1 * GW + xb + 1]);
        const int ya = y0 + 1 > 0 ? y0 + 1 : 0, yb = y1 - 1 < GH - 1 ? y1 - 1 : GH - 1;
        for (int yy = ya; yy <= yb; ++yy) {
          if (x0 >= 0) scan(start[yy * GW + x0], start[yy * GW + x0 + 1]);
          if (x1 < GW) scan(start[yy * GW + x1], start[yy * GW + x1 + 1]);
        }
        const float lbn = (float)(r << lb);
        if (lbn * lbn * (1.f - 4e-6f) > best_s) break;
        if (r >= 2) {
          const int side = 2 * r + 1;
          int todo = side * side;
          if (id) {
            const int need = min(((int)(__builtin_sqrtf(best_s) * 1.00001f) >> lb) + 1, 1 << 12);
            todo = (2 * need + 1) * (2 * need + 1) - side * side;
          }
          if (todo * 4 >= GH * GW) {
            scan(0, start[GH * GW]);
            break;
          }
        }
      }
      (void)best_s;
    }
    const int W = w * up;
    int32_t* o = cells + (size_t)n * hw * up * up + (size_t)(y * up) * W + x * up;
    for (int dy = 0; dy < up; ++dy)
      for (int dx = 0; dx < up; ++dx) o[(size_t)dy * W + dx] = id;
    return;
  }
  float best = (K > 20) ? 1e5f : INFINITY;
  float best_s = (K > 20) ? 1e10f : INFINITY;
  int id = 0;
  const int32_t* cn = centers + (size_t)n * max_centers * 2;
  for (int k0 = 0; k0 < K; k0 += CTR_TILE) {
    const int kn = min(CTR_TILE, K - k0);
    __syncthreads();
    for (int t = threadIdx.x; t < kn; t += 256) {
      cy[t] = (float)(cn[2 * (k0 + t)] * step);
      cx[t] = (float)(cn[2 * (k0 + t) + 1] * step);
    }
    __syncthreads();
    if (active) {
      for (int t = 0; t < kn; ++t) {
        const float dy = cy[t] - ly, dx = cx[t] - lx;
        const float dy2 = dy * dy;
        const float s = __builtin_fmaf(dx, dx, dy2);
        if (s > best_s) continue;
        const float d = __builtin_sqrtf(s);
        const bool first = (K <= 20) && (k0 + t == 0);
        if (d < best || first) { best = d; best_s = s; id = k0 + t + 1; }
      }
    }
  }
  if (!active) return;
  const int W = w * up;
  int32_t* o = cells + (size_t)n * hw * up * up + (size_t)(y * up) * W + x * up;
  for (int dy = 0; dy < up; ++dy)
    for (int dx = 0; dx < up; ++dx) o[(size_t)dy * W + dx] = id;
}

struct ThingList { int32_t n; int32_t cls[16]; };

__device__ __forceinline__ int harden(const float* __restrict__ sem, int C, int64_t plane, int64_t pix, float thr) {
  if (C == 1) return sem[pix] >= thr ? 1 : 0;
  int best = 0;
  float bv = sem[pix];
  for (int c = 1; c < C; ++c) {
    float v = sem[c * plane + pix];
    if (v > bv) { bv = v; best = c; }
  }
  return best;
}
__device__ __forceinline__ bool is_thing(const ThingList& tl, int cls) {
  bool r = false;
  for (int i = 0; i < tl.n; ++i) r |= (tl.cls[i] == cls);
  return r;
}

__global__ void __launch_bounds__(256) merge_count_kernel(const float* __restrict__ sem, const int32_t* __restrict__ cells,
                                                          int C, int CLS, int64_t plane, float thr, ThingList tl,
                                                          int max_ids, int32_t* __restrict__ counts_all,
                                                          size_t img_stride_i32) {
  __shared__ int tkey[256];
  __shared__ int tval[256];
  const int n = blockIdx.y;
  const float* s = sem + (size_t)n * C * plane;
  const int32_t* ce = cells + (size_t)n * plane;
  int32_t* counts = counts_all + (size_t)n * img_stride_i32;
  tkey[threadIdx.x] = -1;
  tval[threadIdx.x] = 0;
  __syncthreads();
  const int stuff_base = (max_ids + 1) * CLS;
  const int64_t p0 = ((int64_t)blockIdx.x * 256 + threadIdx.x) * 8;
  int run_key = -1, run_cnt = 0;
  auto flush = [&]() {
    if (run_cnt == 0) return;
    unsigned h = ((unsigned)run_key * 2654435761u) >> 24;
    bool done = false;
    for (int probe = 0; probe < 256 && !done; ++probe) {
      int old = atomicCAS(&tkey[h], -1, run_key);
      if (old == -1 || old == run_key) {
        atomicAdd(&tval[h], run_cnt);
        done = true;
      } else {
        h = (h + 1) & 255u;
      }
    }
    if (!done) atomicAdd(&counts[run_key], run_cnt);
    run_cnt = 0;
  };
  for (int j = 0; j < 8; ++j) {
    int64_t p = p0 + j;
    if (p >= plane) break;
    int cls = harden(s, C, plane, p, thr);
    int id = is_thing(tl, cls) ? ce[p] : 0;
    if (id > max_ids || id < 0) id = 0;
    int key = id > 0 ? id * CLS + cls : stuff_base + cls;
    if (key != run_key) { flush(); run_key = key; }
    ++run_cnt;
  }
  flush();
  __syncthreads();
  const int k = tkey[threadIdx.x];
  if (k >= 0) atomicAdd(&counts[k], tval[threadIdx.x]);
}

__global__ void __launch_bounds__(256) merge_assign_kernel(int CLS, int max_ids, int64_t divisor,
                                                           int32_t* __restrict__ counts_all,
                                                           int64_t* __restrict__ map_all, size_t img_stride_i32,
                                                           size_t map_stride) {
  __shared__ int cls_of[256];
  __shared__ int run[32];
  const int n = blockIdx.x;
  const int32_t* counts = counts_all + (size_t)n * img_stride_i32;
  int64_t* map = map_all + (size_t)n * map_stride;
  if (threadIdx.x < 32) run[threadIdx.x] = 1;
  __syncthreads();
  for (int id0 = 1; id0 <= max_ids; id0 += 256) {
    const int id = id0 + threadIdx.x;
    int cls = -1;
    if (id <= max_ids) {
      int bc = 0;
      for (int c = 0; c < CLS; ++c) {
        int v = counts[id * CLS + c];
        if (v > bc) { bc = v; cls = c; }
      }
    }
    cls_of[threadIdx.x] = cls;
    __syncthreads();
    if (cls >= 0) {
      int rank = 0;
      for (int t = 0; t < (int)threadIdx.x; ++t) rank += (cls_of[t] == cls);
      map[id] = (int64_t)cls * divisor + (int64_t)(run[cls] + rank);
    } else if (id <= max_ids) {
      map[id] = -1;
    }
    __syncthreads();
    if (threadIdx.x < CLS && threadIdx.x < 32) {
      int tot = 0;
      for (int t = 0; t < 256; ++t) tot += (cls_of[t] == (int)threadIdx.x);
      run[threadIdx.x] += tot;
    }
    __syncthreads();
  }
}

__global__ void __launch_bounds__(256) merge_write_kernel(const float* __restrict__ sem, const int32_t* __restrict__ cells,
                                                          int C, int CLS, int64_t plane, float thr, ThingList tl,
                                                          int max_ids, int64_t divisor, int64_t stuff_area,
                                                          int64_t void_label, const int32_t* __restrict__ stuff_all,
                                                          const int64_t* __restrict__ map_all, size_t img_stride_i32,
                                                          size_t map_stride, int64_t* __restrict__ pan) {
  const int n = blockIdx.y;
  const float* s = sem + (size_t)n * C * plane;
  const int32_t* ce = cells + (size_t)n * plane;
  const int32_t* stuff = stuff_all + (size_t)n * img_stride_i32;
  const int64_t* map = map_all + (size_t)n * map_stride;
  int64_t* o = pan + (size_t)n * plane;
  for (int64_t p = (int64_t)blockIdx.x * 256 + threadIdx.x; p < plane; p += (int64_t)gridDim.x * 256) {
    int cls = harden(s, C, plane, p, thr);
    int64_t v = void_label;
    if (is_thing(tl, cls)) {
      int id = ce[p];
      if (id > 0 && id <= max_ids) {
        int64_t m = map[id];
        if (m >= 0) v = m;
      }
    } else if ((int64_t)stuff[cls] >= stuff_area) {
      v = (int64_t)cls * divisor;
    }
    o[p] = v;
  }
}

}
}

using namespace emp;

extern "C" {

int emp_logits_to_prob(const float* d_logits, float* d_prob, int N, int C, int H, int W, void* stream) {
  hipStream_t s = (hipStream_t)stream;
  EMP_REQUIRE(N > 0 && C > 0 && H > 0 && W > 0, "logits_to_prob: bad shape");
  const int64_t plane = (int64_t)H * W;
  if (C == 1) {
    int64_t total = (int64_t)N * plane;
    hipLaunchKernelGGL(sigmoid_kernel, dim3(grid_for(total)), dim3(256), 0, s, d_logits, d_prob, total);
  } else {
    int64_t total = (int64_t)N * plane;
    hipLaunchKernelGGL(softmax_kernel, dim3(grid_for(total)), dim3(256), 0, s, d_logits, d_prob, C, plane, total);
  }
  EMP_LAUNCH_CHECK();
  return EMP_OK;
}

int emp_median_slices(const float* const* h_slice_ptrs, int ks, float* d_out, size_t count, void* stream) {
  EMP_REQUIRE(ks >= 1 && ks <= MAX_KS && (ks & 1), "median: kernel size %d must be odd and <= %d", ks, MAX_KS);
  MedianPtrs ptrs;
  for (int k = 0; k < MAX_KS; ++k) ptrs.p[k] = k < ks ? h_slice_ptrs[k] : h_slice_ptrs[0];
  hipLaunchKernelGGL(median_kernel, dim3(grid_for((int64_t)count)), dim3(256), 0, (hipStream_t)stream, ptrs, ks, d_out,
                     count);
  EMP_LAUNCH_CHECK();
  return EMP_OK;
}

int emp_median_recursive(const float* d_hist, const float* d_raw, int n_raw, int ks, int n_out, float* d_out,
                         size_t count, void* stream) {
  EMP_REQUIRE(d_hist && d_raw && d_out && count > 0, "median_recursive: null argument");
  EMP_REQUIRE((ks & 1) && ks >= 3 && ks <= MAX_KS, "median_recursive: kernel size %d must be odd, 3..%d", ks, MAX_KS);
  EMP_REQUIRE(n_out >= 1 && n_raw >= n_out + (ks - 1) / 2, "median_recursive: need n_out + mid raw maps");
  hipStream_t s = (hipStream_t)stream;
  const int grid = grid_for((int64_t)count);
  switch (ks) {
    case 3: hipLaunchKernelGGL(median_recursive_kernel<3>, dim3(grid), dim3(256), 0, s, d_hist, d_raw, n_out, d_out, count); break;
    case 5: hipLaunchKernelGGL(median_recursive_kernel<5>, dim3(grid), dim3(256), 0, s, d_hist, d_raw, n_out, d_out, count); break;
    case 7: hipLaunchKernelGGL(median_recursive_kernel<7>, dim3(grid), dim3(256), 0, s, d_hist, d_raw, n_out, d_out, count); break;
    case 9: hipLaunchKernelGGL(median_recursive_kernel<9>, dim3(grid), dim3(256), 0, s, d_hist, d_raw, n_out, d_out, count); break;
    case 11: hipLaunchKernelGGL(median_recursive_kernel<11>, dim3(grid), dim3(256), 0, s, d_hist, d_raw, n_out, d_out, count); break;
    case 13: hipLaunchKernelGGL(median_recursive_kernel<13>, dim3(grid), dim3(256), 0, s, d_hist, d_raw, n_out, d_out, count); break;
    default: hipLaunchKernelGGL(median_recursive_kernel<15>, dim3(grid), dim3(256), 0, s, d_hist, d_raw, n_out, d_out, count); break;
  }
  EMP_LAUNCH_CHECK();
  return EMP_OK;
}

static inline size_t cells_mask_bytes(int N, int h, int w) {
  const size_t words = ((size_t)h * w + 31) / 32 + 2;
  return ((size_t)N * words * 4 + 255) & ~(size_t)255;
}
size_t emp_instance_cells_work_bytes(int N, int h, int w) {
  return cells_mask_bytes(N, h, w) + (size_t)N * GRID_IMG_BYTES + 256;
}

int emp_instance_cells(const float* d_ctr_hmp, const float* d_offsets, int N, int h, int w, float nms_threshold,
                       int nms_kernel, int step, int up, int32_t* d_cells, int32_t* d_centers, int32_t* d_num_centers,
                       int max_centers, void* d_work, void* stream) {
  hipStream_t s = (hipStream_t)stream;
  EMP_REQUIRE(N > 0 && h > 0 && w > 0 && nms_kernel >= 1 && up >= 1 && max_centers > 0, "instance_cells: bad args");
  const int hw = h * w;
  const int words = (hw + 31) / 32 + 2;
  uint32_t* mask = (uint32_t*)d_work;
  const int nb = cdiv(hw, 256);
  hipLaunchKernelGGL(nms_mask_kernel, dim3(nb, N), dim3(256), 0, s, d_ctr_hmp, h, w, nms_threshold, nms_kernel, mask,
                     words);
  EMP_LAUNCH_CHECK();
  hipLaunchKernelGGL(centers_kernel, dim3(N), dim3(256), 0, s, mask, words, (hw + 31) / 32, w, d_centers,
                     d_num_centers, max_centers);
  EMP_LAUNCH_CHECK();
  const char* grid_env = getenv("EMP_VOTE_GRID");
  char* gridbuf = nullptr;
  if (!(grid_env && grid_env[0] == '0') && (int64_t)h * step < (1 << 20) && (int64_t)w * step < (1 << 20)) {
    gridbuf = (char*)d_work + cells_mask_bytes(N, h, w);
    hipLaunchKernelGGL(ctr_grid_build_kernel, dim3(N), dim3(1024), 0, s, d_centers, d_num_centers, max_centers, step, h * step, w * step, gridbuf);
    EMP_LAUNCH_CHECK();
  }
  hipLaunchKernelGGL(group_pixels_kernel, dim3(nb, N), dim3(256), 0, s, d_offsets, h, w, d_centers, d_num_centers,
                     max_centers, step, up, d_cells, gridbuf);
  EMP_LAUNCH_CHECK();
  return EMP_OK;
}

static inline size_t merge_img_stride_i32(int CLS, int max_ids) {
  size_t n = (size_t)(max_ids + 1) * CLS + CLS;
  return (n + 3) & ~(size_t)3;
}
size_t emp_panoptic_merge_work_bytes(int N, int C, int max_ids) {
  const int CLS = C < 2 ? 2 : C;
  return (size_t)N * (merge_img_stride_i32(CLS, max_ids) * 4 + (size_t)(max_ids + 1) * 8) + 256;
}

int emp_panoptic_merge(const float* d_sem, const int32_t* d_cells, int N, int C, int H, int W, float confidence_thr,
                       const int32_t* h_thing_list, int n_things, int64_t label_divisor, int64_t stuff_area,
                       int64_t void_label, int max_ids, int64_t* d_pan, void* d_work, void* stream) {
  hipStream_t s = (hipStream_t)stream;
  EMP_REQUIRE(N > 0 && C > 0 && C <= 32 && H > 0 && W > 0 && max_ids >= 0, "panoptic_merge: bad args");
  EMP_REQUIRE(n_things >= 0 && n_things <= 16, "panoptic_merge: at most 16 thing classes");
  const int CLS = C < 2 ? 2 : C;
  ThingList tl;
  tl.n = n_things;
  for (int i = 0; i < 16; ++i) tl.cls[i] = i < n_things ? h_thing_list[i] : -1;
  const size_t stride = merge_img_stride_i32(CLS, max_ids);
  int32_t* counts = (int32_t*)d_work;
  int32_t* stuff = counts + (size_t)(max_ids + 1) * CLS;
  int64_t* map = (int64_t*)((char*)d_work + (((size_t)N * stride * 4 + 15) & ~(size_t)15));
  const size_t map_stride = (size_t)max_ids + 1;
  EMP_CHECK_HIP(hipMemsetAsync(d_work, 0, (size_t)N * stride * 4, s));
  const int64_t plane = (int64_t)H * W;
  const int nb = (int)cdiv64(plane, 256 * 8);
  hipLaunchKernelGGL(merge_count_kernel, dim3(nb, N), dim3(256), 0, s, d_sem, d_cells, C, CLS, plane, confidence_thr,
                     tl, max_ids, counts, stride);
  EMP_LAUNCH_CHECK();
  hipLaunchKernelGGL(merge_assign_kernel, dim3(N), dim3(256), 0, s, CLS, max_ids, label_divisor, counts, map, stride,
                     map_stride);
  EMP_LAUNCH_CHECK();
  hipLaunchKernelGGL(merge_write_kernel, dim3(grid_for(plane, 256, 2048), N), dim3(256), 0, s, d_sem, d_cells, C, CLS,
                     plane, confidence_thr, tl, max_ids, label_divisor, stuff_area, void_label, stuff, map, stride,
                     map_stride, d_pan);
  EMP_LAUNCH_CHECK();
  return EMP_OK;
}

}
```

### include/empanada_hip.h

```cpp
#ifndef EMPANADA_HIP_H
#define EMPANADA_HIP_H

#include <stddef.h>
#include <stdint.h>

#if defined(__GNUC__)
#define EMP_API __attribute__((visibility("default")))
#else
#define EMP_API
#endif

#ifdef __cplusplus
extern "C" {
#endif

typedef enum {
  EMP_OK = 0,
  EMP_ERR_INVALID = -1,
  EMP_ERR_HIP = -2,
  EMP_ERR_STATE = -3,
  EMP_ERR_NOMEM = -4
} emp_status;

EMP_API const char* emp_last_error(void);
// ... 91 lines not shown

EMP_API int emp_conv2d_nhwc_f16x3_ex(const float* d_in, int N, int H, int W, int Cin, int in_ld,
                        const float* d_w, const float* d_bias, const float* d_bias_n,
                        const float* d_res, int res_ld,
                        void* d_out, int out_ld, int out_fmt, int Cout,
                        int KH, int KW, int stride, int pad, int dil, int act, int wmode,
                        const float* d_in2, int H2, int W2, int Cin2, int in2_ld, int stride2,
                        const float* d_head_w, const float* d_head_b, int head_c, float* d_head_out,
                        void* stream);

EMP_API int emp_hl32_from_f32(const float* d_in, void* d_out, int64_t rows, int C, int in_ld, int out_ld, void* stream);
EMP_API int emp_hl32_to_f32(const void* d_in, float* d_out, int64_t rows, int C, int in_ld, int out_ld, void* stream);
EMP_API int emp_x3p_pack_weights(const float* d_w, void* d_img, int Cout, int K, void* stream);
EMP_API int emp_conv2d_hl32_f16x3(const void* d_in, int N, int H, int W, int Cin, int in_ld,
                        const void* d_wimg, const float* d_bias, const float* d_bias_n,
                        const void* d_res, int res_ld, int res_fmt,
                        void* d_out, int out_ld, int out_fmt, int Cout,
                        int KH, int KW, int stride, int pad, int dil, int act, void* stream);
EMP_API int emp_conv2d_hl32_f16x3_ksplit(const void* d_in, int N, int H, int W, int Cin, int in_ld,
                        const void* d_wimg, const float* d_bias, const float* d_bias_n,
                        const void* d_res, int res_ld, int res_fmt,
                        void* d_out, int out_ld, int out_fmt, void* d_out2, int out2_ld, int split2, int Cout,
                        int KH, int KW, int stride, int pad, int dil, int act,
                        void* d_scratch, int64_t scratch_bytes, void* stream);

EMP_API int emp_sepconv_x3_pack(const float* d_dw, const float* d_pw, int ks, int C, int Cout,
                        float* d_dw_packed, void* d_pw_packed, void* stream);
EMP_API int emp_sepconv_x3_nhwc_f32(const float* d_in, int N, int H, int W, int C, int in_ld,
                        const float* d_dw_packed, const void* d_pw_packed, const float* d_bias, int Cout, int act,
                        float* d_out, int out_ld,
                        const float* d_head_w, const float* d_head_b, int head_c, float* d_head_out,
                        int ks, void* stream);

EMP_API int emp_conv2d_grouped_nhwc_f32(const float* d_in, int N, int H, int W, int groups, int cin_g, int Cin16, int in_ld,
                        const float* d_w, const float* d_bias, float* d_out, int out_ld, int cout_g,
                        int KH, int KW, int stride, int pad, int dil, int act, void* stream);

EMP_API int emp_conv1x1_dual_nhwc_f16(const void* d_in, int N, int H, int W, int Cin, int in_ld, const void* d_in2,
                              int H2, int W2, int Cin2, int in2_ld, int stride2, const void* d_w,
                              const float* d_bias, void* d_out, int out_ld, int Cout, int relu, int variant,
                              void* stream);

EMP_API int emp_dwconv_nhwc_f16(const void* d_in, int N, int H, int W, int C, int in_ld,
                        const void* d_w, int K, void* d_out, int out_ld, void* stream);

EMP_API int emp_sepconv5x5_pack_pw(const void* d_pw_w, int pw_ld, int C, int Cout, void* d_packed, void* stream);
EMP_API int emp_sepconv5x5_nhwc_f16(const void* d_in, int N, int H, int W, int C, int in_ld,
                        const void* d_dw_w, const void* d_pw_w, const float* d_bias,
                        int Cout, int act, void* d_out, int out_ld,
                        const float* d_head_w, const float* d_head_b, int head_c, float* d_head_out,
                        void* stream);
EMP_API int emp_sepconv3x3_nhwc_f16(const void* d_in, int N, int H, int W, int C, int in_ld, const void* d_dw_w,
                            const void* d_pw_w, const float* d_bias, int Cout, int act, void* d_out, int out_ld,
                            void* stream);

EMP_API int emp_sepconvp_pack_dw(const void* d_dw_w, int K, int C, void* d_packed, void* stream);
EMP_API int emp_sepconvp_pack_pw(const void* d_pw_w, int pw_ld, int C, int Cout, void* d_packed, void* stream);
EMP_API int emp_sepconvp_nhwc_f16(const void* d_in, int N, int H, int W, int C, int in_ld, int K,
                        const void* d_dw_w, const void* d_pw_w, const float* d_bias,
                        int Cout, int act, void* d_out, int out_ld,
                        const float* d_head_w, const float* d_head_b, int head_c, float* d_head_out,
                        void* stream);
EMP_API int emp_sepconvp_ws_pack_pw(const void* d_pw_w, int pw_ld, int C, int Cout, void* d_packed, void* stream);
EMP_API int emp_sepconvp_ws_nhwc_f16(const void* d_in, int N, int H, int W, int C, int in_ld, int K,
                        const void* d_dw_w, const void* d_pw_w, const float* d_bias,
                        int Cout, int act, void* d_out, int out_ld,
                        const float* d_head_w, const float* d_head_b, int head_c, float* d_head_out,
                        void* stream);


EMP_API int emp_logits_to_prob(const float* d_logits, float* d_prob, int N, int C, int H, int W, void* stream);

EMP_API int emp_median_slices(const float* const* h_slice_ptrs, int ks, float* d_out,
                      size_t count, void* stream);

EMP_API int emp_median_recursive(const float* d_hist, const float* d_raw, int n_raw, int ks, int n_out,
                         float* d_out, size_t count, void* stream);

EMP_API size_t emp_instance_cells_work_bytes(int N, int h, int w);
EMP_API int emp_instance_cells(const float* d_ctr_hmp, const float* d_offsets, int N, int h, int w,
                       float nms_threshold, int nms_kernel, int step, int up,
                       int32_t* d_cells, int32_t* d_centers, int32_t* d_num_centers,
                       int max_centers, void* d_work, void* stream);

EMP_API size_t emp_panoptic_merge_work_bytes(int N, int C, int max_ids);
EMP_API int emp_panoptic_merge(const float* d_sem, const int32_t* d_cells, int N, int C, int H, int W,
                       float confidence_thr, const int32_t* h_thing_list, int n_things,
                       int64_t label_divisor, int64_t stuff_area, int64_t void_label,
                       int max_ids, int64_t* d_pan, void* d_work, void* stream);


EMP_API size_t emp_ccl8_work_bytes(int N, int H, int W);
EMP_API int emp_ccl8(const int32_t* d_in, int N, int H, int W, int32_t* d_out, int32_t* d_num,
             void* d_work, void* stream);

EMP_API size_t emp_force_connected_work_bytes(int N, int H, int W);
EMP_API int emp_force_connected(const int64_t* d_pan, int N, int H, int W, const int32_t* h_thing_list, int n_things,
                        int64_t label_divisor, int32_t* d_out, void* d_work, void* stream);

EMP_API int emp_ccl26(const int32_t* d_in, int D, int H, int W, int32_t* d_out, int32_t* d_num,
              void* d_work, void* stream);

EMP_API int emp_morph_cross3d(const uint32_t* d_in, uint32_t* d_out, int D, int H, int W, int op, void* stream);

EMP_API int emp_fill_holes_slices(uint32_t* h_vol, int64_t D, int64_t H, int64_t W);

EMP_API size_t emp_rle_extract_work_bytes(int N, int H, int W);
EMP_API int emp_rle_extract(const int32_t* d_labels, int N, int H, int W, int32_t* d_runs,
                    int32_t* d_num_runs, int max_runs, void* d_work, void* stream);

EMP_API int emp_ccl_range(const void* d_in, int in_bytes, int N, int depth, int H, int W, int64_t lo, int64_t hi,
                        int32_t* d_out, int32_t* d_num, void* d_work, void* stream);
EMP_API int emp_rle_extract_range(const void* d_labels, int in_bytes, int N, int H, int W, int64_t lo, int64_t hi,
                        int32_t* d_runs, int32_t* d_num_runs, int max_runs, void* d_work, void* stream);

EMP_API int emp_rle_fill(const int64_t* d_starts, const int64_t* d_lens, const int64_t* d_vals,
                 int64_t nruns, void* d_volume, int64_t size, int elem_bytes, void* stream);

EMP_API int emp_rle_fill_ordered(const int64_t* d_starts, const int64_t* d_lens, const int64_t* d_vals,
                 const int32_t* d_order, int64_t nruns, void* d_volume, int64_t size, int elem_bytes,
                 int32_t* d_prio, void* stream);

EMP_API int emp_rle_pair_intersections(const int64_t* h_starts, const int64_t* h_runs, const int64_t* h_off,
                               const int64_t* h_pairs, int64_t n_pairs, int64_t* h_out);
EMP_API int emp_ranges_vote(const int64_t* h_ranges, int64_t n, int thr, int64_t* h_out, int64_t* n_out);
EMP_API int emp_gather_segments_i64(const int64_t* const* h_src_a, const int64_t* const* h_src_b, const int32_t* h_src_id,
                            const int64_t* h_src_off, const int64_t* h_cnt, const int64_t* h_out_off, int64_t n_seg,
                            int64_t* h_out_a, int64_t* h_out_b);

typedef struct emp_stack_matcher emp_stack_matcher_t;
EMP_API emp_stack_matcher_t* emp_sm_create(int64_t class_id, int64_t label_divisor, double iou_thr, double ioa_thr,
                                   int do_match);
EMP_API void emp_sm_destroy(emp_stack_matcher_t* h);
EMP_API int emp_sm_push_slice_runs(emp_stack_matcher_t* h, const int64_t* h_runs, int64_t n, int64_t width, int64_t id_offset);
EMP_API int emp_sm_push_slices_runs(emp_stack_matcher_t* h, int64_t count, const int64_t* const* runs, const int64_t* n,
                                    int64_t width, int64_t id_offset);
EMP_API int emp_sm_push_slice_objects(emp_stack_matcher_t* h, int64_t n, const int64_t* labels, const int64_t* boxes,
                              const int64_t* off, const int64_t* starts, const int64_t* runs);
EMP_API int64_t emp_sm_num_slices(const emp_stack_matcher_t* h);
EMP_API int emp_lsa_maximize(const double* cost, int64_t nr, int64_t nc, int64_t* rows, int64_t* cols);
EMP_API int emp_lsa_maximize_sparse(int64_t nr, int64_t nc, int64_t nnz, const int64_t* er, const int64_t* ec, const double* ew,
                                    int64_t* rows, int64_t* cols);
EMP_API int emp_sm_prepare(emp_stack_matcher_t* h, int64_t from, int64_t to);
EMP_API int emp_sm_state_size(const emp_stack_matcher_t* h, int64_t idx, int64_t* n_obj, int64_t* n_mem);
EMP_API int emp_sm_export_state(const emp_stack_matcher_t* h, int64_t idx, int64_t* labels, int64_t* off, int64_t* members,
                                int64_t* next_label);
EMP_API int emp_sm_import_state(emp_stack_matcher_t* h, int64_t idx, int64_t n_obj, const int64_t* labels, const int64_t* off,
                                const int64_t* members, int64_t next_label, int assign_new);
EMP_API int emp_sm_begin_backward(emp_stack_matcher_t* h);
EMP_API int emp_sm_step_begin(emp_stack_matcher_t* h, int64_t idx, int* nt, int* nm);
EMP_API const double* emp_sm_iou(const emp_stack_matcher_t* h);
EMP_API int emp_sm_step_apply(emp_stack_matcher_t* h, const int64_t* rows, const int64_t* cols, int64_t n);
EMP_API int emp_sm_run(emp_stack_matcher_t* h, int64_t idx, int dir, int64_t count, int track, int64_t* stopped_at);
EMP_API int emp_sm_solver_stats(const emp_stack_matcher_t* h, int64_t* sparse_steps, int64_t* dense_steps);
EMP_API int emp_sm_pending_shape(const emp_stack_matcher_t* h, int* nt, int* nm);
EMP_API int emp_sm_tracker_init(emp_stack_matcher_t* h, int axis , int64_t D, int64_t H, int64_t W);
EMP_API int emp_sm_track(emp_stack_matcher_t* h, int64_t idx, int64_t index2d);
EMP_API int emp_sm_track_range(emp_stack_matcher_t* h, int64_t first, int64_t last, int64_t global_first);
EMP_API int emp_sm_tracker_finish(emp_stack_matcher_t* h);
EMP_API int64_t emp_sm_num_tracks(const emp_stack_matcher_t* h);
EMP_API int emp_sm_track_info(const emp_stack_matcher_t* h, int64_t k, int64_t* label, int64_t* box6, int64_t* n_runs);
EMP_API int emp_sm_track_runs(const emp_stack_matcher_t* h, int64_t k, int64_t* starts, int64_t* runs);
EMP_API int emp_sm_tracks_info(const emp_stack_matcher_t* h, int64_t* labels, int64_t* boxes6, int64_t* counts, int64_t* total_runs);
EMP_API int emp_sm_tracks_runs(const emp_stack_matcher_t* h, int64_t* starts, int64_t* runs);
EMP_API int64_t emp_sm_slice_num_objects(const emp_stack_matcher_t* h, int64_t idx);
EMP_API int emp_sm_slice_object_info(const emp_stack_matcher_t* h, int64_t idx, int64_t k, int64_t* label, int64_t* box4,
// ... 50 lines not shown
```

Before: 1342.

## Fuse PointRend upsample with radix-select top-k and vectorize panoptic merge

```diff
diff --git a/empanada-napari_amd/_abi.py b/empanada-napari_amd/_abi.py
--- a/empanada-napari_amd/_abi.py
+++ b/empanada-napari_amd/_abi.py
@@ -119,6 +119,8 @@
     'emp_instance_cells_work_bytes': (sz, [c_int, c_int, c_int]),
     'emp_instance_cells': (c_int, [vp, vp, c_int, c_int, c_int, c_f32, c_int, c_int, c_int, vp, vp, vp, c_int, vp, vp]),
     'emp_panoptic_merge_work_bytes': (sz, [c_int, c_int, c_int]),
+    'emp_pr_select_work_bytes': (sz, [c_int, c_int, c_int]),
+    'emp_pr_select': (c_int, [vp, c_int, c_int, c_int, c_int, c_int, c_int, vp, vp, vp, sz, vp]),
     'emp_ccl8_work_bytes': (sz, [c_int, c_int, c_int]),
     'emp_ccl8': (c_int, [vp, c_int, c_int, c_int, vp, vp, vp, vp]),
     'emp_force_connected_work_bytes': (sz, [c_int, c_int, c_int]),
diff --git a/empanada-napari_amd/csrc/abi.hip b/empanada-napari_amd/csrc/abi.hip
--- a/empanada-napari_amd/csrc/abi.hip
+++ b/empanada-napari_amd/csrc/abi.hip
@@ -64,6 +64,24 @@
   EMP_REQUIRE(d_dst && d_src, "copy_d2d: null pointer");
   EMP_CHECK_HIP(hipMemcpyAsync(d_dst, d_src, bytes, hipMemcpyDeviceToDevice, (hipStream_t)stream));
   return EMP_OK;
+}
+
+static inline size_t pr_select_keys_bytes(int N, int h, int w) { return ((size_t)N * 4 * h * w * 4 + 255) & ~(size_t)255; }
+size_t emp_pr_select_work_bytes(int N, int h, int w) {
+  return pr_select_keys_bytes(N, h, w) + topk_work_bytes(N, (int64_t)4 * h * w);
+}
+
+int emp_pr_select(const float* d_in, int N, int C, int h, int w, int k, int mode, float* d_out, int32_t* d_idx, void* d_work,
+                  size_t work_bytes, void* stream) {
+  EMP_REQUIRE(d_in && d_out && d_idx && d_work, "pr_select: null pointer");
+  EMP_REQUIRE(N > 0 && C >= 1 && C <= 8 && h > 0 && w > 0 && (int64_t)N * 4 * h * w < ((int64_t)1 << 31), "pr_select: bad shape");
+  EMP_REQUIRE(mode == 0 || mode == 1, "pr_select: mode %d", mode);
+  EMP_REQUIRE(work_bytes >= emp_pr_select_work_bytes(N, h, w), "pr_select: workspace too small");
+  const size_t kb = pr_select_keys_bytes(N, h, w);
+  char* topk = (char*)d_work + kb;
+  if (mode == 1) return launch_upsample2x_select(d_in, N, C, h, w, k, d_out, topk, work_bytes - kb, d_idx, (hipStream_t)stream);
+  if (int rc = launch_upsample2x_keys(d_in, N, C, h, w, d_out, (uint32_t*)d_work, (hipStream_t)stream)) return rc;
+  return launch_topk_smallest((const uint32_t*)d_work, N, (int64_t)4 * h * w, k, topk, work_bytes - kb, d_idx, (hipStream_t)stream);
 }
 
 int emp_conv2d_nhwc_f16(const void* d_in, int N, int H, int W, int Cin, int in_ld, const void* d_w,
diff --git a/empanada-napari_amd/csrc/common.h b/empanada-napari_amd/csrc/common.h
--- a/empanada-napari_amd/csrc/common.h
+++ b/empanada-napari_amd/csrc/common.h
@@ -194,6 +194,8 @@
 
 size_t topk_work_bytes(int N, int64_t plane);
 int launch_upsample2x_keys(const float* in, int N, int C, int h, int w, float* out, uint32_t* keys, hipStream_t s);
+int launch_upsample2x_select(const float* in, int N, int C, int h, int w, int k, float* out, void* work,
+                             size_t work_bytes, int32_t* idx_out, hipStream_t s);
 int launch_topk_smallest(const uint32_t* keys, int N, int64_t plane, int k, void* work, size_t work_bytes,
                          int32_t* idx_out, hipStream_t s);
 int launch_point_features(const half_t* feat, int N, int fh, int fw, int C, int feat_ld, const float* coarse,
diff --git a/empanada-napari_amd/csrc/pdl_net.hip b/empanada-napari_amd/csrc/pdl_net.hip
--- a/empanada-napari_amd/csrc/pdl_net.hip
+++ b/empanada-napari_amd/csrc/pdl_net.hip
@@ -111,6 +111,7 @@
   int64_t par_limit = [] { const char* e = getenv("EMP_PAR_DECODERS"); return e ? atoll(e) : (int64_t)4 << 20; }();
   hipStream_t aux = nullptr;
   hipEvent_t ev_fork = nullptr, ev_join = nullptr;
+  bool pr_select = [] { const char* e = getenv("EMP_PR_SELECT"); return !(e && e[0] == '0'); }();
 
   ~emp_pdl() {
     for (void* p : owned) (void)hipFree(p);
@@ -609,7 +610,7 @@
       plane_max = (int64_t)hh * ww;
     }
   }
-  add_raw(n, pl, "pr.keys", (size_t)N * plane_max * 4);
+  if (!n->pr_select) add_raw(n, pl, "pr.keys", (size_t)N * plane_max * 4);
   add_raw(n, pl, "pr.topk", topk_work_bytes(N, plane_max));
   add_raw(n, pl, "pr.idx", (size_t)N * P * 4);
   add_raw(n, pl, "pr.x0", (size_t)N * P * ldp * 2);
@@ -1160,16 +1161,20 @@
   const float* coarse = head_out[0];
   const float* cur = coarse;
   int hh = hq, ww = wq;
-  uint32_t* keys = rawp<uint32_t>(n, "pr.keys");
+  uint32_t* keys = n->pr_select ? nullptr : rawp<uint32_t>(n, "pr.keys");
   int32_t* idx = rawp<int32_t>(n, "pr.idx");
   half_t* X[2] = {rawp<half_t>(n, "pr.x0"), rawp<half_t>(n, "pr.x1")};
   for (int st = 0; st < RS; ++st) {
     float* nxt = (st + 1 < RS) ? rawp<float>(n, "pr.sem" + std::to_string(st)) : o_sem;
-    RC(launch_upsample2x_keys(cur, N, n->ncls, hh, ww, nxt, keys, s));
+    const int64_t plane = (int64_t)hh * ww * 4;
+    const int k = (int)(plane < P ? plane : P);
+    if (n->pr_select) {
+      RC(launch_upsample2x_select(cur, N, n->ncls, hh, ww, k, nxt, rawp<char>(n, "pr.topk"), n->raw.at("pr.topk").second, idx, s));
+    } else {
+      RC(launch_upsample2x_keys(cur, N, n->ncls, hh, ww, nxt, keys, s));
+      RC(launch_topk_smallest(keys, N, plane, k, rawp<char>(n, "pr.topk"), n->raw.at("pr.topk").second, idx, s));
+    }
     hh *= 2; ww *= 2;
-    const int64_t plane = (int64_t)hh * ww;
-    const int k = (int)(plane < P ? plane : P);
-    RC(launch_topk_smallest(keys, N, plane, k, rawp<char>(n, "pr.topk"), n->raw.at("pr.topk").second, idx, s));
     if (n->fuse_pr && pr_mlp_supported(n->dec_ch, ldp, n->ncls, c.num_fc)) {
       const half_t* fw_[4];
       const float* fb_[4];
@@ -1980,8 +1985,8 @@
   int hh = hq, ww = wq;
   int64_t plane_max = (int64_t)hq * wq;
   for (int st = 0; st < RS; ++st) plane_max *= 4;
-  float* fkeys;
-  RC32(buf32(n, "pr.keys", (size_t)N * plane_max, &fkeys));
+  float* fkeys = nullptr;
+  if (!n->pr_select) RC32(buf32(n, "pr.keys", (size_t)N * plane_max, &fkeys));
   float* ftopk;
   const size_t topk_bytes = topk_work_bytes(N, plane_max);
   RC32(buf32(n, "pr.topk", (topk_bytes + 3) / 4, &ftopk));
@@ -1995,11 +2000,15 @@
   for (int st = 0; st < RS; ++st) {
     float* nxt = o_sem;
     if (st + 1 < RS) RC32(buf32(n, "pr.sem" + std::to_string(st), (size_t)N * n->ncls * hh * ww * 4, &nxt));
-    RC32(launch_upsample2x_keys(cur, N, n->ncls, hh, ww, nxt, (uint32_t*)fkeys, s));
+    const int64_t plane = (int64_t)hh * ww * 4;
+    const int k = (int)(plane < P ? plane : P);
+    if (n->pr_select) {
+      RC32(launch_upsample2x_select(cur, N, n->ncls, hh, ww, k, nxt, (char*)ftopk, topk_bytes, (int32_t*)fidx, s));
+    } else {
+      RC32(launch_upsample2x_keys(cur, N, n->ncls, hh, ww, nxt, (uint32_t*)fkeys, s));
+      RC32(launch_topk_smallest((const uint32_t*)fkeys, N, plane, k, (char*)ftopk, topk_bytes, (int32_t*)fidx, s));
+    }
     hh *= 2; ww *= 2;
-    const int64_t plane = (int64_t)hh * ww;
-    const int k = (int)(plane < P ? plane : P);
-    RC32(launch_topk_smallest((const uint32_t*)fkeys, N, plane, k, (char*)ftopk, topk_bytes, (int32_t*)fidx, s));
     RC32(launch_point_features_f32(semx.p, N, hq, wq, n->dec_ch, semx.ld, coarse, n->ncls, (const int32_t*)fidx, k, hh, ww, X[0].p,
                                    X[1].p, ldp, s));
     T32 xa[2] = {X[0], X[1]};
diff --git a/empanada-napari_amd/csrc/pointrend.hip b/empanada-napari_amd/csrc/pointrend.hip
--- a/empanada-napari_amd/csrc/pointrend.hip
+++ b/empanada-napari_amd/csrc/pointrend.hip
@@ -25,6 +25,35 @@
     if (i < w) base += sh[i];
   *total = sh[0] + sh[1] + sh[2] + sh[3];
   return base + inc - v;
+}
+
+__device__ __forceinline__ void up2_axis(int o, int size, int& i0, int& i1, float& lo, float& hi) {
+  float f = 0.5f * ((float)o + 0.5f) - 0.5f;
+  f = f < 0.f ? 0.f : f;
+  i0 = (int)f;
+  i1 = i0 + (i0 < size - 1 ? 1 : 0);
+  lo = f - (float)i0;
+  hi = 1.f - lo;
+}
+__device__ __forceinline__ float up2_sample(float b00, float b01, float b10, float b11, float hx, float lx, float hy,
+                                            float ly) {
+#pragma clang fp contract(off)
+  const float t0 = hx * b00;
+  const float t1 = lx * b11;
+  const float top = __builtin_fmaf(lx, b01, t0);
+  const float bot = __builtin_fmaf(hx, b10, t1);
+  const float a = hy * top;
+  const float b = ly * bot;
+  return a + b;
+}
+__device__ __forceinline__ uint32_t pr_key(const float (&v)[8], int C) {
+  float top1 = -INFINITY, top2 = -INFINITY;
+#pragma unroll
+  for (int c = 0; c < 8; ++c)
+    if (c < C) {
+      if (v[c] > top1) { top2 = top1; top1 = v[c]; } else if (v[c] > top2) { top2 = v[c]; }
+    }
+  return __float_as_uint((C == 1) ? fabsf(v[0]) : (top1 - top2));
 }
 
 __global__ void __launch_bounds__(256) upsample2x_keys_kernel(const float* __restrict__ in, int N, int C, int h, int w,
@@ -36,25 +65,248 @@
     int64_t p = i / W;
     int oy = (int)(p % H);
     int n = (int)(p / H);
-    float fy = 0.5f * ((float)oy + 0.5f) - 0.5f;
-    float fx = 0.5f * ((float)ox + 0.5f) - 0.5f;
-    fy = fy < 0.f ? 0.f : fy;
-    fx = fx < 0.f ? 0.f : fx;
-    int y0 = (int)fy, x0 = (int)fx;
-    int y1 = y0 + (y0 < h - 1 ? 1 : 0), x1 = x0 + (x0 < w - 1 ? 1 : 0);
-    float ly = fy - (float)y0, lx = fx - (float)x0;
-    float hy = 1.f - ly, hx = 1.f - lx;
-    float top1 = -INFINITY, top2 = -INFINITY, v0 = 0.f;
-    for (int c = 0; c < C; ++c) {
-      const float* b = in + ((size_t)n * C + c) * h * w;
-      float v = hy * (hx * b[y0 * w + x0] + lx * b[y0 * w + x1]) + ly * (hx * b[y1 * w + x0] + lx * b[y1 * w + x1]);
-      out[(((size_t)n * C + c) * H + oy) * W + ox] = v;
-      if (c == 0) v0 = v;
-      if (v > top1) { top2 = top1; top1 = v; } else if (v > top2) { top2 = v; }
-    }
-    float key = (C == 1) ? fabsf(v0) : (top1 - top2);
-    keys[i] = __float_as_uint(key);
-  }
+    int y0, y1, x0, x1;
+    float ly, hy, lx, hx;
+    up2_axis(oy, h, y0, y1, ly, hy);
+    up2_axis(ox, w, x0, x1, lx, hx);
+    float v[8] = {0.f, 0.f, 0.f, 0.f, 0.f, 0.f, 0.f, 0.f};
+#pragma unroll
+    for (int c = 0; c < 8; ++c)
+      if (c < C) {
+        const float* b = in + ((size_t)n * C + c) * h * w;
+        v[c] = up2_sample(b[y0 * w + x0], b[y0 * w + x1], b[y1 * w + x0], b[y1 * w + x1], hx, lx, hy, ly);
+        out[(((size_t)n * C + c) * H + oy) * W + ox] = v[c];
+      }
+    keys[i] = pr_key(v, C);
+  }
+}
+
+constexpr int L1_BINS = 2048;
+constexpr int HCHUNK = 8192;
+
+__device__ __forceinline__ void wave_hist_add(uint32_t* lh, uint32_t packed, bool active) {
+  const int lane = threadIdx.x & 63;
+  bool pending = active;
+  while (__ballot(pending)) {
+    if (pending) {
+      const uint32_t lead = (uint32_t)__builtin_amdgcn_readfirstlane((int)packed);
+      const bool match = packed == lead;
+      const uint64_t m = __ballot(match);
+      if (match) {
+        if (lane == __ffsll((unsigned long long)m) - 1) atomicAdd(&lh[lead & (L1_BINS - 1)], (uint32_t)__popcll(m) * (lead >> 16));
+        pending = false;
+      }
+    }
+  }
+}
+
+template <int VW>
+__global__ void __launch_bounds__(256) upsample2x_hist_kernel(const float* __restrict__ in, int C, int h, int w,
+                                                              float* __restrict__ out, uint32_t* __restrict__ hist) {
+  __shared__ uint32_t lh[L1_BINS];
+  const int H = 2 * h, W = 2 * w;
+  const int n = blockIdx.y;
+  const int nq = (W + 3) >> 2;
+  const int64_t items = (int64_t)H * nq;
+  if (hist) {
+    for (int b = threadIdx.x; b < L1_BINS; b += 256) lh[b] = 0;
+    __syncthreads();
+  }
+  const float* src = in + (size_t)n * C * h * w;
+  float* dst = out + (size_t)n * C * H * W;
+  const int64_t step = (int64_t)gridDim.x * 256;
+  for (int64_t it0 = (int64_t)blockIdx.x * 256; it0 < items; it0 += step) {
+    const int64_t it = it0 + threadIdx.x;
+    const bool live = it < items;
+    const int oy = live ? (int)(it / nq) : 0;
+    const int ox = live ? (int)(it - (int64_t)oy * nq) * 4 : 0;
+    const int nv = !live ? 0 : (W - ox < 4 ? W - ox : 4);
+    int y0, y1;
+    float ly, hy;
+    up2_axis(oy, h, y0, y1, ly, hy);
+    float v[4][8];
+#pragma unroll
+    for (int j = 0; j < 4; ++j)
+#pragma unroll
+      for (int c = 0; c < 8; ++c) v[j][c] = 0.f;
+    if (live) {
+#pragma unroll
+      for (int j = 0; j < 4; ++j) {
+        if (j < nv) {
+          int x0, x1;
+          float lx, hx;
+          up2_axis(ox + j, w, x0, x1, lx, hx);
+#pragma unroll
+          for (int c = 0; c < 8; ++c)
+            if (c < C) {
+              const float* b = src + (size_t)c * h * w;
+              v[j][c] = up2_sample(b[y0 * w + x0], b[y0 * w + x1], b[y1 * w + x0], b[y1 * w + x1], hx, lx, hy, ly);
+            }
+        }
+      }
+#pragma unroll
+      for (int c = 0; c < 8; ++c)
+        if (c < C) {
+          float* o = dst + ((size_t)c * H + oy) * W + ox;
+          if (VW == 4) {
+            *reinterpret_cast<float4*>(o) = make_float4(v[0][c], v[1][c], v[2][c], v[3][c]);
+          } else if (VW == 2) {
+            *reinterpret_cast<float2*>(o) = make_float2(v[0][c], v[1][c]);
+            if (nv == 4) *reinterpret_cast<float2*>(o + 2) = make_float2(v[2][c], v[3][c]);
+          } else {
+#pragma unroll
+            for (int j = 0; j < 4; ++j)
+              if (j < nv) o[j] = v[j][c];
+          }
+        }
+    }
+    if (hist) {
+      uint32_t bin[4], cnt[4];
+#pragma unroll
+      for (int j = 0; j < 4; ++j) {
+        bin[j] = (pr_key(v[j], C) >> 20) & (L1_BINS - 1);
+        cnt[j] = j < nv ? 1u : 0u;
+      }
+#pragma unroll
+      for (int j = 3; j > 0; --j)
+        if (cnt[j] && bin[j] == bin[j - 1]) { cnt[j - 1] += cnt[j]; cnt[j] = 0; }
+#pragma unroll
+      for (int j = 0; j < 4; ++j) wave_hist_add(lh, bin[j] | (cnt[j] << 16), cnt[j] != 0);
+    }
+  }
+  if (hist) {
+    __syncthreads();
+    for (int b = threadIdx.x; b < L1_BINS; b += 256) {
+      const uint32_t c = lh[b];
+      if (c) atomicAdd(&hist[(size_t)n * L1_BINS + b], c);
+    }
+  }
+}
+
+template <bool VEC>
+__device__ __forceinline__ void quad_keys(const float* __restrict__ img, int C, int64_t plane, int64_t e,
+                                          uint32_t (&key)[4]) {
+  float v[4][8];
+#pragma unroll
+  for (int c = 0; c < 8; ++c) {
+    if (c < C) {
+      const float* b = img + (size_t)c * plane;
+      if (VEC) {
+        const float4 t = *reinterpret_cast<const float4*>(b + e);
+        v[0][c] = t.x; v[1][c] = t.y; v[2][c] = t.z; v[3][c] = t.w;
+      } else {
+#pragma unroll
+        for (int j = 0; j < 4; ++j) v[j][c] = e + j < plane ? b[e + j] : 0.f;
+      }
+    } else {
+#pragma unroll
+      for (int j = 0; j < 4; ++j) v[j][c] = 0.f;
+    }
+  }
+#pragma unroll
+  for (int j = 0; j < 4; ++j) key[j] = pr_key(v[j], C);
+}
+
+__global__ void init_select_kernel(uint32_t* state, uint32_t* hist, int N, uint32_t k) {
+  int i = blockIdx.x * 256 + threadIdx.x;
+  if (i < N) { state[4 * i] = 0; state[4 * i + 1] = k; state[4 * i + 2] = 0; state[4 * i + 3] = 0; }
+  if (i < N * L1_BINS) hist[i] = 0;
+}
+
+template <bool VEC>
+__global__ void __launch_bounds__(256) radix_hist_out_kernel(const float* __restrict__ out, int C, int64_t plane,
+                                                             const uint32_t* __restrict__ state,
+                                                             uint32_t* __restrict__ hist, int shift, uint32_t binmask,
+                                                             uint32_t himask) {
+  __shared__ uint32_t lh[L1_BINS];
+  const int n = blockIdx.y;
+  for (int b = threadIdx.x; b < L1_BINS; b += 256) lh[b] = 0;
+  __syncthreads();
+  const uint32_t prefix = state[4 * n];
+  const float* img = out + (size_t)n * C * plane;
+  const int64_t base = (int64_t)blockIdx.x * HCHUNK;
+  int any = 0;
+#pragma unroll 2
+  for (int j = 0; j < HCHUNK / 1024; ++j) {
+    const int64_t e = base + (int64_t)j * 1024 + threadIdx.x * 4;
+    if (e < plane) {
+      uint32_t key[4];
+      quad_keys<VEC>(img, C, plane, e, key);
+#pragma unroll
+      for (int q = 0; q < 4; ++q)
+        if ((VEC || e + q < plane) && (key[q] & himask) == prefix) {
+          atomicAdd(&lh[(key[q] >> shift) & binmask], 1u);
+          any = 1;
+        }
+    }
+  }
+  if (!__syncthreads_or(any)) return;
+  for (int b = threadIdx.x; b < L1_BINS; b += 256) {
+    const uint32_t c = lh[b];
+    if (c) atomicAdd(&hist[(size_t)n * L1_BINS + b], c);
+  }
+}
+
+template <int PER>
+__global__ void __launch_bounds__(256) radix_select_wide_kernel(uint32_t* __restrict__ hist,
+                                                                uint32_t* __restrict__ state, int shift) {
+  __shared__ uint32_t sh[8];
+  const int n = blockIdx.x;
+  uint32_t* hp = hist + (size_t)n * L1_BINS + threadIdx.x * PER;
+  uint32_t c[PER], sum = 0;
+#pragma unroll
+  for (int j = 0; j < PER; ++j) { c[j] = hp[j]; hp[j] = 0; sum += c[j]; }
+  uint32_t total;
+  uint32_t ex = block_excl_scan(sum, sh, &total);
+  const uint32_t krem = state[4 * n + 1];
+  const uint32_t prefix = state[4 * n];
+  __syncthreads();
+#pragma unroll
+  for (int j = 0; j < PER; ++j) {
+    if (c[j] > 0 && ex < krem && krem <= ex + c[j]) {
+      state[4 * n] = prefix | ((uint32_t)(threadIdx.x * PER + j) << shift);
+      state[4 * n + 1] = krem - ex;
+    }
+    ex += c[j];
+  }
+}
+
+template <bool VEC>
+__device__ __forceinline__ uint32_t count_flags_out(const float* __restrict__ img, int C, int64_t plane, int64_t e0,
+                                                    uint32_t T, uint32_t* flags_less, uint32_t* flags_eq) {
+  uint32_t fl = 0, fe = 0;
+#pragma unroll
+  for (int g = 0; g < 2; ++g) {
+    const int64_t e = e0 + 4 * g;
+    if (e < plane) {
+      uint32_t key[4];
+      quad_keys<VEC>(img, C, plane, e, key);
+#pragma unroll
+      for (int q = 0; q < 4; ++q)
+        if (VEC || e + q < plane) {
+          fl |= (uint32_t)(key[q] < T) << (4 * g + q);
+          fe |= (uint32_t)(key[q] == T) << (4 * g + q);
+        }
+    }
+  }
+  *flags_less = fl;
+  *flags_eq = fe;
+  return (uint32_t)__popc(fl) | ((uint32_t)__popc(fe) << 16);
+}
+
+template <bool VEC>
+__global__ void __launch_bounds__(256) compact_count_out_kernel(const float* __restrict__ out, int C, int64_t plane,
+                                                                const uint32_t* __restrict__ state,
+                                                                uint32_t* __restrict__ blockcnt, int nb) {
+  __shared__ uint32_t sh[8];
+  const int n = blockIdx.y;
+  const uint32_t T = state[4 * n];
+  uint32_t fl, fe;
+  uint32_t c = count_flags_out<VEC>(out + (size_t)n * C * plane, C, plane,
+                                    (int64_t)blockIdx.x * CHUNK + threadIdx.x * 8, T, &fl, &fe);
+  uint32_t total;
+  block_excl_scan(c, sh, &total);
+  if (threadIdx.x == 0) blockcnt[(size_t)n * nb + blockIdx.x] = total;
 }
 
 __global__ void init_state_kernel(uint32_t* state, uint32_t* hist, int N, uint32_t k) {
@@ -154,6 +406,24 @@
   }
 }
 
+__device__ __forceinline__ void compact_emit(uint32_t c, uint32_t fl, uint32_t fe, int64_t e0, uint32_t krem, int k,
+                                             const uint32_t* __restrict__ blockoff, int nb, int n, uint32_t* sh,
+                                             int32_t* __restrict__ idx_out) {
+  const uint32_t nless = (uint32_t)k - krem;
+  uint32_t tl, te;
+  uint32_t pl = block_excl_scan(c & 0xffffu, sh, &tl) + blockoff[((size_t)n * nb + blockIdx.x) * 2];
+  uint32_t pe = block_excl_scan(c >> 16, sh, &te) + blockoff[((size_t)n * nb + blockIdx.x) * 2 + 1];
+  int32_t* o = idx_out + (size_t)n * k;
+#pragma unroll
+  for (int j = 0; j < 8; ++j) {
+    if (fl & (1u << j)) { o[pl++] = (int32_t)(e0 + j); }
+    if (fe & (1u << j)) {
+      if (pe < krem) o[nless + pe] = (int32_t)(e0 + j);
+      ++pe;
+    }
+  }
+}
+
 __global__ void __launch_bounds__(256) compact_write_kernel(const uint32_t* __restrict__ keys, int64_t plane,
                                                             const uint32_t* __restrict__ state,
                                                             const uint32_t* __restrict__ blockoff, int nb, int k,
@@ -161,23 +431,24 @@
   __shared__ uint32_t sh[8];
   const int n = blockIdx.y;
   const uint32_t T = state[4 * n];
-  const uint32_t krem = state[4 * n + 1];
-  const uint32_t nless = (uint32_t)k - krem;
   const int64_t e0 = (int64_t)blockIdx.x * CHUNK + threadIdx.x * 8;
   uint32_t fl, fe;
   uint32_t c = count_flags(keys + (size_t)n * plane, plane, e0, T, &fl, &fe);
-  uint32_t tl, te;
-  uint32_t pl = block_excl_scan(c & 0xffffu, sh, &tl) + blockoff[((size_t)n * nb + blockIdx.x) * 2];
-  uint32_t pe = block_excl_scan(c >> 16, sh, &te) + blockoff[((size_t)n * nb + blockIdx.x) * 2 + 1];
-  int32_t* o = idx_out + (size_t)n * k;
-#pragma unroll
-  for (int j = 0; j < 8; ++j) {
-    if (fl & (1u << j)) { o[pl++] = (int32_t)(e0 + j); }
-    if (fe & (1u << j)) {
-      if (pe < krem) o[nless + pe] = (int32_t)(e0 + j);
-      ++pe;
-    }
-  }
+  compact_emit(c, fl, fe, e0, state[4 * n + 1], k, blockoff, nb, n, sh, idx_out);
+}
+
+template <bool VEC>
+__global__ void __launch_bounds__(256) compact_write_out_kernel(const float* __restrict__ out, int C, int64_t plane,
+                                                                const uint32_t* __restrict__ state,
+                                                                const uint32_t* __restrict__ blockoff, int nb, int k,
+                                                                int32_t* __restrict__ idx_out) {
+  __shared__ uint32_t sh[8];
+  const int n = blockIdx.y;
+  const uint32_t T = state[4 * n];
+  const int64_t e0 = (int64_t)blockIdx.x * CHUNK + threadIdx.x * 8;
+  uint32_t fl, fe;
+  uint32_t c = count_flags_out<VEC>(out + (size_t)n * C * plane, C, plane, e0, T, &fl, &fe);
+  compact_emit(c, fl, fe, e0, state[4 * n + 1], k, blockoff, nb, n, sh, idx_out);
 }
 
 __global__ void iota_kernel(int32_t* idx, int N, int k) {
@@ -477,7 +748,78 @@
 
 size_t topk_work_bytes(int N, int64_t plane) {
   int nb = (int)cdiv64(plane, CHUNK);
-  return (size_t)N * (256 + 4 + (size_t)nb * 3) * sizeof(uint32_t) + 256;
+  return (size_t)N * (L1_BINS + 4 + (size_t)nb * 3) * sizeof(uint32_t) + 256;
+}
+
+int launch_upsample2x_select(const float* in, int N, int C, int h, int w, int k, float* out, void* work,
+                             size_t work_bytes, int32_t* idx_out, hipStream_t s) {
+  EMP_REQUIRE(C >= 1 && C <= 8 && N > 0 && h > 0 && w > 0, "pr_select: bad shape N=%d C=%d h=%d w=%d", N, C, h, w);
+  const int H = 2 * h, W = 2 * w;
+  const int64_t plane = (int64_t)H * W;
+  EMP_REQUIRE(k > 0 && (int64_t)k <= plane, "pr_select: k=%d plane=%lld", k, (long long)plane);
+  const bool all = (int64_t)k == plane;
+  EMP_REQUIRE(all || work_bytes >= topk_work_bytes(N, plane), "pr_select: workspace too small");
+  const int nb = (int)cdiv64(plane, CHUNK);
+  uint32_t* hist = (uint32_t*)work;
+  uint32_t* state = hist + (size_t)N * L1_BINS;
+  uint32_t* blockcnt = state + (size_t)N * 4;
+  uint32_t* blockoff = blockcnt + (size_t)N * nb;
+  if (!all) {
+    hipLaunchKernelGGL(init_select_kernel, dim3(cdiv(N * L1_BINS, 256)), dim3(256), 0, s, state, hist, N, (uint32_t)k);
+    EMP_LAUNCH_CHECK();
+  }
+  {
+    const int64_t items = (int64_t)H * ((W + 3) / 4);
+    int cap = 2048 / N;
+    if (cap < 1) cap = 1;
+    const dim3 grid(grid_for(items, 256, cap), N);
+    uint32_t* hp = all ? nullptr : hist;
+    const uintptr_t a = (uintptr_t)out;
+    if (W % 4 == 0 && a % 16 == 0)
+      hipLaunchKernelGGL(upsample2x_hist_kernel<4>, grid, dim3(256), 0, s, in, C, h, w, out, hp);
+    else if (a % 8 == 0)
+      hipLaunchKernelGGL(upsample2x_hist_kernel<2>, grid, dim3(256), 0, s, in, C, h, w, out, hp);
+    else
+      hipLaunchKernelGGL(upsample2x_hist_kernel<1>, grid, dim3(256), 0, s, in, C, h, w, out, hp);
+    EMP_LAUNCH_CHECK();
+  }
+  if (all) {
+    hipLaunchKernelGGL(iota_kernel, dim3(cdiv(N * k, 256)), dim3(256), 0, s, idx_out, N, k);
+    EMP_LAUNCH_CHECK();
+    return EMP_OK;
+  }
+  const bool vec = plane % 4 == 0 && (uintptr_t)out % 16 == 0;
+  const int nbh = (int)cdiv64(plane, HCHUNK);
+  hipLaunchKernelGGL(radix_select_wide_kernel<8>, dim3(N), dim3(256), 0, s, hist, state, 20);
+  EMP_LAUNCH_CHECK();
+  for (int level = 2; level <= 3; ++level) {
+    const int shift = level == 2 ? 9 : 0;
+    const uint32_t binmask = level == 2 ? 2047u : 511u;
+    const uint32_t himask = level == 2 ? 0xfff00000u : 0xfffffe00u;
+    if (vec)
+      hipLaunchKernelGGL(radix_hist_out_kernel<true>, dim3(nbh, N), dim3(256), 0, s, out, C, plane, state, hist, shift, binmask, himask);
+    else
+      hipLaunchKernelGGL(radix_hist_out_kernel<false>, dim3(nbh, N), dim3(256), 0, s, out, C, plane, state, hist, shift, binmask, himask);
+    EMP_LAUNCH_CHECK();
+    if (level == 2)
+      hipLaunchKernelGGL(radix_select_wide_kernel<8>, dim3(N), dim3(256), 0, s, hist, state, shift);
+    else
+      hipLaunchKernelGGL(radix_select_wide_kernel<2>, dim3(N), dim3(256), 0, s, hist, state, shift);
+    EMP_LAUNCH_CHECK();
+  }
+  if (vec)
+    hipLaunchKernelGGL(compact_count_out_kernel<true>, dim3(nb, N), dim3(256), 0, s, out, C, plane, state, blockcnt, nb);
+  else
+    hipLaunchKernelGGL(compact_count_out_kernel<false>, dim3(nb, N), dim3(256), 0, s, out, C, plane, state, blockcnt, nb);
+  EMP_LAUNCH_CHECK();
+  hipLaunchKernelGGL(compact_scan_kernel, dim3(N), dim3(256), 0, s, blockcnt, blockoff, nb);
+  EMP_LAUNCH_CHECK();
+  if (vec)
+    hipLaunchKernelGGL(compact_write_out_kernel<true>, dim3(nb, N), dim3(256), 0, s, out, C, plane, state, blockoff, nb, k, idx_out);
+  else
+    hipLaunchKernelGGL(compact_write_out_kernel<false>, dim3(nb, N), dim3(256), 0, s, out, C, plane, state, blockoff, nb, k, idx_out);
+  EMP_LAUNCH_CHECK();
+  return EMP_OK;
 }
 
 int launch_topk_smallest(const uint32_t* keys, int N, int64_t plane, int k, void* work, size_t work_bytes,
diff --git a/empanada-napari_amd/csrc/postprocess.hip b/empanada-napari_amd/csrc/postprocess.hip
--- a/empanada-napari_amd/csrc/postprocess.hip
+++ b/empanada-napari_amd/csrc/postprocess.hip
@@ -356,6 +356,25 @@
   }
   return best;
 }
+__device__ __forceinline__ void harden4(const float* __restrict__ sem, int C, int64_t plane, int64_t pix, float thr,
+                                        int* cls) {
+  const float4 a = *reinterpret_cast<const float4*>(sem + pix);
+  float bv[4] = {a.x, a.y, a.z, a.w};
+  if (C == 1) {
+#pragma unroll
+    for (int j = 0; j < 4; ++j) cls[j] = bv[j] >= thr ? 1 : 0;
+    return;
+  }
+#pragma unroll
+  for (int j = 0; j < 4; ++j) cls[j] = 0;
+  for (int c = 1; c < C; ++c) {
+    const float4 b = *reinterpret_cast<const float4*>(sem + c * plane + pix);
+    const float v[4] = {b.x, b.y, b.z, b.w};
+#pragma unroll
+    for (int j = 0; j < 4; ++j)
+      if (v[j] > bv[j]) { bv[j] = v[j]; cls[j] = c; }
+  }
+}
 __device__ __forceinline__ bool is_thing(const ThingList& tl, int cls) {
   bool r = false;
   for (int i = 0; i < tl.n; ++i) r |= (tl.cls[i] == cls);
@@ -365,7 +384,7 @@
 __global__ void __launch_bounds__(256) merge_count_kernel(const float* __restrict__ sem, const int32_t* __restrict__ cells,
                                                           int C, int CLS, int64_t plane, float thr, ThingList tl,
                                                           int max_ids, int32_t* __restrict__ counts_all,
-                                                          size_t img_stride_i32) {
+                                                          size_t img_stride_i32, int vec) {
   __shared__ int tkey[256];
   __shared__ int tval[256];
   const int n = blockIdx.y;
@@ -394,15 +413,33 @@
     if (!done) atomicAdd(&counts[run_key], run_cnt);
     run_cnt = 0;
   };
-  for (int j = 0; j < 8; ++j) {
-    int64_t p = p0 + j;
-    if (p >= plane) break;
-    int cls = harden(s, C, plane, p, thr);
-    int id = is_thing(tl, cls) ? ce[p] : 0;
+  auto visit = [&](int cls, int id) {
+    if (!is_thing(tl, cls)) id = 0;
     if (id > max_ids || id < 0) id = 0;
     int key = id > 0 ? id * CLS + cls : stuff_base + cls;
     if (key != run_key) { flush(); run_key = key; }
     ++run_cnt;
+  };
+  if (vec) {
+#pragma unroll
+    for (int g = 0; g < 2; ++g) {
+      const int64_t p = p0 + 4 * g;
+      if (p >= plane) break;
+      int cls[4];
+      harden4(s, C, plane, p, thr, cls);
+      const int4 id = *reinterpret_cast<const int4*>(ce + p);
+      visit(cls[0], id.x);
+      visit(cls[1], id.y);
+      visit(cls[2], id.z);
+      visit(cls[3], id.w);
+    }
+  } else {
+    for (int j = 0; j < 8; ++j) {
+      int64_t p = p0 + j;
+      if (p >= plane) break;
+      int cls = harden(s, C, plane, p, thr);
+      visit(cls, is_thing(tl, cls) ? ce[p] : 0);
+    }
   }
   flush();
   __syncthreads();
@@ -455,18 +492,16 @@
                                                           int max_ids, int64_t divisor, int64_t stuff_area,
                                                           int64_t void_label, const int32_t* __restrict__ stuff_all,
                                                           const int64_t* __restrict__ map_all, size_t img_stride_i32,
-                                                          size_t map_stride, int64_t* __restrict__ pan) {
+                                                          size_t map_stride, int64_t* __restrict__ pan, int vec) {
   const int n = blockIdx.y;
   const float* s = sem + (size_t)n * C * plane;
   const int32_t* ce = cells + (size_t)n * plane;
   const int32_t* stuff = stuff_all + (size_t)n * img_stride_i32;
   const int64_t* map = map_all + (size_t)n * map_stride;
   int64_t* o = pan + (size_t)n * plane;
-  for (int64_t p = (int64_t)blockIdx.x * 256 + threadIdx.x; p < plane; p += (int64_t)gridDim.x * 256) {
-    int cls = harden(s, C, plane, p, thr);
+  auto label = [&](int cls, int id) {
     int64_t v = void_label;
     if (is_thing(tl, cls)) {
-      int id = ce[p];
       if (id > 0 && id <= max_ids) {
         int64_t m = map[id];
         if (m >= 0) v = m;
@@ -474,7 +509,26 @@
     } else if ((int64_t)stuff[cls] >= stuff_area) {
       v = (int64_t)cls * divisor;
     }
-    o[p] = v;
+    return v;
+  };
+  if (vec) {
+    for (int64_t p = ((int64_t)blockIdx.x * 256 + threadIdx.x) * 4; p < plane; p += (int64_t)gridDim.x * 1024) {
+      int cls[4];
+      harden4(s, C, plane, p, thr, cls);
+      const int4 id = *reinterpret_cast<const int4*>(ce + p);
+      longlong2 lo, hi;
+      lo.x = label(cls[0], id.x);
+      lo.y = label(cls[1], id.y);
+      hi.x = label(cls[2], id.z);
+      hi.y = label(cls[3], id.w);
+      *reinterpret_cast<longlong2*>(o + p) = lo;
+      *reinterpret_cast<longlong2*>(o + p + 2) = hi;
+    }
+    return;
+  }
+  for (int64_t p = (int64_t)blockIdx.x * 256 + threadIdx.x; p < plane; p += (int64_t)gridDim.x * 256) {
+    int cls = harden(s, C, plane, p, thr);
+    o[p] = label(cls, is_thing(tl, cls) ? ce[p] : 0);
   }
 }
 
@@ -593,15 +647,16 @@
   EMP_CHECK_HIP(hipMemsetAsync(d_work, 0, (size_t)N * stride * 4, s));
   const int64_t plane = (int64_t)H * W;
   const int nb = (int)cdiv64(plane, 256 * 8);
+  const int vec = plane % 4 == 0 && (((uintptr_t)d_sem | (uintptr_t)d_cells | (uintptr_t)d_pan) & 15) == 0;
   hipLaunchKernelGGL(merge_count_kernel, dim3(nb, N), dim3(256), 0, s, d_sem, d_cells, C, CLS, plane, confidence_thr,
-                     tl, max_ids, counts, stride);
+                     tl, max_ids, counts, stride, vec);
   EMP_LAUNCH_CHECK();
   hipLaunchKernelGGL(merge_assign_kernel, dim3(N), dim3(256), 0, s, CLS, max_ids, label_divisor, counts, map, stride,
                      map_stride);
   EMP_LAUNCH_CHECK();
-  hipLaunchKernelGGL(merge_write_kernel, dim3(grid_for(plane, 256, 2048), N), dim3(256), 0, s, d_sem, d_cells, C, CLS,
-                     plane, confidence_thr, tl, max_ids, label_divisor, stuff_area, void_label, stuff, map, stride,
-                     map_stride, d_pan);
+  hipLaunchKernelGGL(merge_write_kernel, dim3(grid_for(vec ? plane / 4 : plane, 256, 2048), N), dim3(256), 0, s, d_sem,
+                     d_cells, C, CLS, plane, confidence_thr, tl, max_ids, label_divisor, stuff_area, void_label, stuff,
+                     map, stride, map_stride, d_pan, vec);
   EMP_LAUNCH_CHECK();
   return EMP_OK;
 }
diff --git a/include/empanada_hip.h b/include/empanada_hip.h
--- a/include/empanada_hip.h
+++ b/include/empanada_hip.h
@@ -197,6 +197,10 @@
                        float nms_threshold, int nms_kernel, int step, int up,
                        int32_t* d_cells, int32_t* d_centers, int32_t* d_num_centers,
                        int max_centers, void* d_work, void* stream);
+
+EMP_API size_t emp_pr_select_work_bytes(int N, int h, int w);
+EMP_API int emp_pr_select(const float* d_in, int N, int C, int h, int w, int k, int mode, float* d_out, int32_t* d_idx,
+                          void* d_work, size_t work_bytes, void* stream);
 
 EMP_API size_t emp_panoptic_merge_work_bytes(int N, int C, int max_ids);
 EMP_API int emp_panoptic_merge(const float* d_sem, const int32_t* d_cells, int N, int C, int H, int W,
```

Result: slower. 1321 (-1.6%).
